# marl/l3embedding

Hardware: AMD Instinct MI355X
Metric: AVC training pairs/sec (1s audio + 224x224 frame) (higher is better)
Workload: dtype f32; 1 GPU; full cnn_L3_melspec2 AVC training step (audio+vision+fusion, fwd+bwd+Adam), batch 64 per GPU, global batch 64, fp32, inputs resident in HBM; global_batch=64, parallelism=dp1, fp32_conv=f4x4

## Files before the change

include/l3hip.h:

```cpp
#ifndef L3HIP_H
#define L3HIP_H

#include <stdint.h>

#ifdef __cplusplus
extern "C" {
#endif

#define L3_OK 0
#define L3_EINVAL (-1)
#define L3_EHIP (-2)
#define L3_ENOMEM (-3)
#define L3_ESTATE (-4)
#define L3_ECOMM (-5)

#define L3_MODEL_CNN_L3_ORIG 0
#define L3_MODEL_TINY_L3 1
#define L3_MODEL_CNN_L3_KAPREDBINPUTBN 2
#define L3_MODEL_CNN_L3_MELSPEC1 3
#define L3_MODEL_CNN_L3_MELSPEC2 4

typedef struct l3_engine l3_engine;

#define L3_DTYPE_F32 0
// ... 37 lines not shown
int l3_copy_state(l3_engine *dst, l3_engine *src);
int l3_optimizer_steps(const l3_engine *e, int64_t *adam_t, int64_t *bn_steps);

int l3_forward(l3_engine *e, const float *video, const float *audio, int training,
               float *probs, float *logits);

int l3_train_step(l3_engine *e, const float *video, const float *audio,
                  const float *labels, float lr, float *loss, float *acc);
int l3_eval_step(l3_engine *e, const float *video, const float *audio,
                 const float *labels, float *loss, float *acc);

int l3_upload_batch(l3_engine *e, const float *video, const float *audio, const float *labels);
int l3_upload_batch_raw(l3_engine *e, const uint8_t *video_u8, const int16_t *audio_i16,
                        const int32_t *labels_i32);
int l3_stage_batch_raw(l3_engine *e, const uint8_t *video_u8, const int16_t *audio_i16, const int32_t *labels_i32);
typedef struct l3_augment_params {
    int32_t start_x, start_y;
    int32_t flip;
    int32_t sat_first;
    float saturation;
    float brightness;
} l3_augment_params;
int l3_upload_batch_raw_aug(l3_engine *e, const uint8_t *video_u8, const int16_t *audio_i16, const int32_t *labels_i32,
                            const l3_augment_params *params, const double *u);
int l3_stage_batch_raw_aug(l3_engine *e, const uint8_t *video_u8, const int16_t *audio_i16, const int32_t *labels_i32,
                           const l3_augment_params *params, const double *u);
int l3_batch_gains(l3_engine *e, double *gains);
int l3_step_forward(l3_engine *e, int training);
int l3_tower_step(l3_engine *e, int tower, int backward);
int l3_step_bucket_count(const l3_engine *e);
int l3_step_backward_bucket(l3_engine *e, int bucket);
int l3_step_update(l3_engine *e, float lr, float grad_scale);
int l3_step_resident(l3_engine *e, float lr);
int l3_step_results(l3_engine *e, float *loss, float *acc, float *probs, float *logits);
int l3_step_results_enqueue(l3_engine *e, int slot, int reduce);
int l3_step_results_wait(l3_engine *e, int slot, float *loss, float *acc);

#define L3_COMM_ID_BYTES 128
int l3_comm_unique_id(void *id128);
int l3_comm_init(l3_engine *e, const void *id128, int world, int rank);
int l3_comm_destroy(l3_engine *e);
int l3_comm_info(const l3_engine *e, int *world, int *rank, char *library_path, int path_cap);
int l3_comm_version(void);
int l3_comm_allreduce_host(l3_engine *e, double *vals, int n, int op);
int l3_step_dp(l3_engine *e, float lr);
int l3_comm_timing(l3_engine *e, int on);
int l3_comm_timing_read(l3_engine *e, double *exposed_ms, double *span_ms, double *bucket_ms, int cap, int *steps);

int l3_grad_arena_dev(l3_engine *e, void **dev_ptr, int64_t *numel);
int l3_bucket_range(const l3_engine *e, int bucket, int64_t *offset, int64_t *numel);
int l3_bn_stats_pack_dev(l3_engine *e, void **send_dev, int64_t *numel);
int l3_bn_stats_replicas_dev(l3_engine *e, int world, void **gathered_dev);

int l3_embed_audio(l3_engine *e, const float *audio, int64_t n, int pool_h, int pool_w, float *out);
int l3_embed_vision(l3_engine *e, const float *video, int64_t n, int pool_h, int pool_w, float *out);
int64_t l3_embed_dim(const l3_engine *e, int vision, int pool_h, int pool_w);
int l3_embed_audio_frames(l3_engine *e, const float *samples, int64_t n_samples, const int64_t *table,
                          int64_t n_frames, int pool_h, int pool_w, float *out);
int l3_embed_audio_clips_resampled(l3_engine *e, const float *native, int64_t n_native, const int64_t *clips,
                                   int64_t n_clips, const double *half_window, int64_t n_window, int num_table,
                                   int64_t n_samples, const int64_t *table, int64_t n_frames, int pool_h, int pool_w,
                                   float *out);

int l3_get_activation(l3_engine *e, const char *name, float *dst, int64_t numel);
int l3_activation_numel(l3_engine *e, const char *name, int64_t *numel);
int l3_sync(l3_engine *e);
int l3_profile_enable(l3_engine *e, int on);
int l3_set_tower_overlap(l3_engine *e, int on);
int l3_profile_read(l3_engine *e, int family, double *ms, int64_t *launches, double *flops);
int l3_profile_read_executed(l3_engine *e, int family, double *flops);
int l3_profile_read_bytes(l3_engine *e, int family, double *bytes);

#define L3_OP_BF16_STORED 2
#define L3_OP_BF16_STORED_OUT 3
int l3_op_conv2d_fwd_dt(int device, int dtype, const float *x, const float *w, const float *b, float *y,
                        int n, int h, int wd, int cin, int cout, int kh, int kw, int same);
int l3_op_conv2d_bwd_dt(int device, int dtype, const float *x, const float *w, const float *dy, float *dx,
                        float *dw, float *db, int n, int h, int wd, int cin, int cout, int kh, int kw, int same);
int l3_op_conv2d_fwd(int device, const float *x, const float *w, const float *b, float *y,
                     int n, int h, int wd, int cin, int cout, int kh, int kw, int same);
int l3_op_conv2d_bwd(int device, const float *x, const float *w, const float *dy,
                     float *dx, float *dw, float *db,
                     int n, int h, int wd, int cin, int cout, int kh, int kw, int same);
int l3_op_bn_relu_fwd(int device, const float *x, const float *gamma, const float *beta,
                      float *y, float *mean, float *var, int64_t rows, int c, int relu, int x_bf16);
int l3_op_bn_relu_bwd(int device, const float *x, const float *y, const float *dy,
                      const float *gamma, const float *beta, const float *mean, const float *var,
                      float *dx, float *dgamma, float *dbeta, int64_t rows, int c, int relu, int x_bf16);
int l3_op_bn_relu_pool2_fwd(int device, const float *x, const float *gamma, const float *beta, float *p,
                            float *mean, float *var, int n, int h, int wd, int c, int same, int relu_mode, int x_bf16);
int l3_op_bn_relu_pool2_bwd(int device, const float *x, const float *gamma, const float *beta, const float *dp,
                            float *dx, float *dgamma, float *dbeta, float *dbias, int n, int h, int wd, int c,
                            int same, int relu_mode, int x_bf16);
int l3_op_maxpool_fwd(int device, const float *x, float *y, int n, int h, int wd, int c,
                      int ph, int pw, int sh, int sw, int same);
int l3_op_maxpool_bwd(int device, const float *x, const float *dy, float *dx, int n, int h,
                      int wd, int c, int ph, int pw, int sh, int sw, int same);
int l3_op_frontend(int device, int model_type, const float *audio, int n, int db_max_scope, float *out);
int l3_op_gather_frames(int device, const float *samples, int64_t n_samples, const int64_t *table,
                        int64_t n_frames, float *frames);
int l3_op_resample(int device, const float *x, int64_t n_in, int64_t sr_orig, int64_t sr_new, const double *half_window,
                   int64_t n_window, int num_table, int64_t t0, int64_t n_out, float *y);
int l3_op_resample_clips(int device, const float *x, int64_t n_in, const int64_t *clips, int64_t n_clips, int64_t sr_new,
                         const double *half_window, int64_t n_window, int num_table, int64_t n_samples, int copy_equal,
                         float *y);
int l3_op_bn_stats_from_partials(int device, const float *part, int nblk, int c, const float *pivot, int64_t rows,
                                 float eps, float *mean, float *var);
int l3_op_preprocess(int device, const uint8_t *video_u8, int64_t nv, float *video,
                     const int16_t *audio_i16, int64_t na, float *audio);
int l3_op_augment_video(int device, const uint8_t *u8, int n, int h, int w, const l3_augment_params *params,
                        uint8_t *out_u8, float *out_f32);
int l3_op_augment_audio(int device, const int16_t *i16, int n, int t, const double *u, int16_t *out_i16, float *out_f32,
                        double *gains);

typedef struct l3_mlp l3_mlp;
int l3_mlp_create(int device, int D, int C, int batch, float weight_decay, uint64_t seed, l3_mlp **m);
void l3_mlp_destroy(l3_mlp *m);
int64_t l3_mlp_param_count(const l3_mlp *m);
int l3_mlp_set_data(l3_mlp *m, const float *X_train, const int32_t *y_train, int64_t n_train,
                    const float *X_valid, const int32_t *y_valid, int64_t n_valid);
int l3_mlp_epoch(l3_mlp *m, const int32_t *perm, float lr, int64_t t0, double *stats_out);
int l3_mlp_predict(l3_mlp *m, const float *X, int64_t n, float *probs_out);
int l3_mlp_get_weights(l3_mlp *m, float *dst, int64_t n);
int l3_mlp_set_weights(l3_mlp *m, const float *src, int64_t n);

int l3_op_mlp_dense_fwd(int device, const float *x, int64_t n_x, const int32_t *idx, int rows, int K, int N, const float *w,
                        const float *b, int relu, float *y);
int l3_op_mlp_dense_bwd_x(int device, const float *dy, const float *w, const float *h, int rows, int K, int N, float *dx);
int l3_op_mlp_wgrad(int device, const float *x, int64_t n_x, const int32_t *idx, int rows, int K, int N, const float *dy, float *dw,
                    float *db);
int l3_op_mlp_wgrad_adam(int device, const float *x, int64_t n_x, const int32_t *idx, int rows, int K, int N, const float *dy,
                         float *w, float *b, float *mw, float *vw, float *mb, float *vb, float weight_decay, float lr_t,
                         float *w2_out);
int l3_op_mlp_softmax_ce(int device, const float *z, const int32_t *labels, int rows, int C, float gscale, float *probs, float *dz,
                         float *ce, float *correct);
int l3_op_adam(int device, float *p, const float *g, float *m, float *v, int64_t n, int64_t n_l2, float l2x2, float lr_t);
int l3_op_adam_scaled(int device, float *p, const float *g, float *m, float *v, int64_t n, int64_t n_l2, float l2x2, float lr_t,
                      float b1, float b2, float eps, float gscale);

int l3_op_head_dense_fwd(int device, const float *x, const float *w, const float *b, float *y, int B, int K, int N, int relu);
int l3_op_head_dense_bwd(int device, const float *x, const float *w, const float *dy, float *dw, float *db, float *dx, int B,
                         int K, int N);
int l3_op_softmax_ce2(int device, const float *logits, const float *labels, int B, float gscale, float *probs, float *dlogits,
                      float *stats);
int l3_op_sumsq(int device, const float *base, int64_t n_base, const int64_t *off, const int64_t *n, int count, int multi,
                float *out);
int l3_op_bn_moving_update(int device, int entries, const int32_t *c, const int64_t *slot_off, int64_t n_slots, float *moving,
                           float *biased, const float *batch, const float *gathered, int64_t n_gathered, int replicas,
                           int64_t stride, float momentum, int zero_debias, int64_t step, float *packed, int64_t n_packed);

#define L3_SVM_LINEAR 0
#define L3_SVM_POLY 1
#define L3_SVM_RBF 2
#define L3_SVM_SIGMOID 3
#define L3_SVM_DEFAULT_WS 64
#define L3_SVM_LOCAL_REL 0.1
typedef struct l3_svm_kernel {
    int32_t kind, degree;
    double gamma, coef0;
} l3_svm_kernel;
typedef struct l3_svm l3_svm;
int l3_svm_create(int device, l3_svm **m);
void l3_svm_destroy(l3_svm *m);
int l3_svm_set_data(l3_svm *m, const float *X, int64_t n, int D);
int l3_svm_fit(l3_svm *m, const l3_svm_kernel *k, double C, double tol, int64_t max_iter, int n_prob, const int64_t *prob_off,
               const int32_t *rows, const int8_t *signs, int q, double *alpha_out, double *rho_out, int64_t *updates_out,
// ... 113 lines not shown
```

l3embedding_amd/_lib.py:

```python
import ctypes as C
import os

import numpy as np

from . import _build

MODEL_IDS = {
    'cnn_L3_orig': 0,
    'tiny_L3': 1,
    'cnn_L3_kapredbinputbn': 2,
    'cnn_L3_melspec1': 3,
    'cnn_L3_melspec2': 4,
}

FAMILIES = ('conv_fwd', 'conv_dgrad', 'conv_wgrad', 'elementwise', 'frontend', 'head', 'adam')


DTYPES = {'f32': 0, 'fp32': 0, 'float32': 0, 'bf16': 1}
FP32_CONV = {'f4x4': 0, 'f2x2': 1, 'f2x2_bf16x6': 2}
DP_MOVING = {'replicas': 0, 'rank_local': 1}
OP_DTYPES = dict(DTYPES, bf16_stored=2, bf16_stored_out=3)


class L3Config(C.Structure):
# ... 10 lines not shown
        ('fp32_conv', C.c_int32),
        ('dp_moving', C.c_int32),
    ]


class L3Error(RuntimeError):
    pass


_f32p = C.POINTER(C.c_float)
_lib = None
TORCH_LOADED_FIRST = None

SIGNATURES = {
    'l3_create': (C.c_int, [C.POINTER(L3Config), C.c_uint64, C.POINTER(C.c_void_p)]),
    'l3_destroy': (None, [C.c_void_p]),
    'l3_last_error': (C.c_char_p, [C.c_void_p]),
    'l3_build_experiments': (C.c_int, []),
    'l3_comm_version': (C.c_int, []),
    'l3_bn_stats_pack_dev': (C.c_int, [C.c_void_p, C.POINTER(C.c_void_p), C.POINTER(C.c_int64)]),
    'l3_bn_stats_replicas_dev': (C.c_int, [C.c_void_p, C.c_int, C.POINTER(C.c_void_p)]),
    'l3_model_type_from_name': (C.c_int, [C.c_char_p]),
    'l3_device_count': (C.c_int, []),
    'l3_param_count': (C.c_int, [C.c_void_p]),
    'l3_param_info': (C.c_int, [C.c_void_p, C.c_int, C.c_char_p, C.c_int, C.POINTER(C.c_int32),
                                C.POINTER(C.c_int64), C.POINTER(C.c_int32), C.POINTER(C.c_int64)]),
    'l3_set_param': (C.c_int, [C.c_void_p, C.c_char_p, C.c_void_p, C.c_int64]),
    'l3_get_param': (C.c_int, [C.c_void_p, C.c_char_p, C.c_void_p, C.c_int64]),
    'l3_get_grad': (C.c_int, [C.c_void_p, C.c_char_p, C.c_void_p, C.c_int64]),
    'l3_reset_optimizer': (C.c_int, [C.c_void_p]),
    'l3_copy_state': (C.c_int, [C.c_void_p, C.c_void_p]),
    'l3_optimizer_steps': (C.c_int, [C.c_void_p, C.POINTER(C.c_int64), C.POINTER(C.c_int64)]),
    'l3_forward': (C.c_int, [C.c_void_p, C.c_void_p, C.c_void_p, C.c_int, C.c_void_p, C.c_void_p]),
    'l3_train_step': (C.c_int, [C.c_void_p, C.c_void_p, C.c_void_p, C.c_void_p, C.c_float,
                                C.POINTER(C.c_float), C.POINTER(C.c_float)]),
    'l3_eval_step': (C.c_int, [C.c_void_p, C.c_void_p, C.c_void_p, C.c_void_p,
                               C.POINTER(C.c_float), C.POINTER(C.c_float)]),
    'l3_upload_batch': (C.c_int, [C.c_void_p, C.c_void_p, C.c_void_p, C.c_void_p]),
    'l3_upload_batch_raw': (C.c_int, [C.c_void_p, C.c_void_p, C.c_void_p, C.c_void_p]),
    'l3_tower_step': (C.c_int, [C.c_void_p, C.c_int, C.c_int]),
    'l3_stage_batch_raw': (C.c_int, [C.c_void_p, C.c_void_p, C.c_void_p, C.c_void_p]),
    'l3_upload_batch_raw_aug': (C.c_int, [C.c_void_p, C.c_void_p, C.c_void_p, C.c_void_p, C.c_void_p, C.c_void_p]),
    'l3_stage_batch_raw_aug': (C.c_int, [C.c_void_p, C.c_void_p, C.c_void_p, C.c_void_p, C.c_void_p, C.c_void_p]),
    'l3_batch_gains': (C.c_int, [C.c_void_p, C.c_void_p]),
    'l3_step_forward': (C.c_int, [C.c_void_p, C.c_int]),
    'l3_step_bucket_count': (C.c_int, [C.c_void_p]),
    'l3_step_backward_bucket': (C.c_int, [C.c_void_p, C.c_int]),
    'l3_step_update': (C.c_int, [C.c_void_p, C.c_float, C.c_float]),
    'l3_step_resident': (C.c_int, [C.c_void_p, C.c_float]),
    'l3_step_results': (C.c_int, [C.c_void_p, C.POINTER(C.c_float), C.POINTER(C.c_float), C.c_void_p, C.c_void_p]),
    'l3_step_results_enqueue': (C.c_int, [C.c_void_p, C.c_int, C.c_int]),
    'l3_step_results_wait': (C.c_int, [C.c_void_p, C.c_int, C.POINTER(C.c_float), C.POINTER(C.c_float)]),
    'l3_comm_unique_id': (C.c_int, [C.c_void_p]),
    'l3_comm_init': (C.c_int, [C.c_void_p, C.c_void_p, C.c_int, C.c_int]),
    'l3_comm_destroy': (C.c_int, [C.c_void_p]),
    'l3_comm_info': (C.c_int, [C.c_void_p, C.POINTER(C.c_int), C.POINTER(C.c_int), C.c_char_p, C.c_int]),
    'l3_comm_allreduce_host': (C.c_int, [C.c_void_p, C.POINTER(C.c_double), C.c_int, C.c_int]),
    'l3_step_dp': (C.c_int, [C.c_void_p, C.c_float]),
    'l3_comm_timing': (C.c_int, [C.c_void_p, C.c_int]),
    'l3_comm_timing_read': (C.c_int, [C.c_void_p, C.POINTER(C.c_double), C.POINTER(C.c_double), C.POINTER(C.c_double), C.c_int, C.POINTER(C.c_int)]),
    'l3_grad_arena_dev': (C.c_int, [C.c_void_p, C.POINTER(C.c_void_p), C.POINTER(C.c_int64)]),
    'l3_bucket_range': (C.c_int, [C.c_void_p, C.c_int, C.POINTER(C.c_int64), C.POINTER(C.c_int64)]),
    'l3_embed_audio': (C.c_int, [C.c_void_p, C.c_void_p, C.c_int64, C.c_int, C.c_int, C.c_void_p]),
    'l3_embed_vision': (C.c_int, [C.c_void_p, C.c_void_p, C.c_int64, C.c_int, C.c_int, C.c_void_p]),
    'l3_embed_dim': (C.c_int64, [C.c_void_p, C.c_int, C.c_int, C.c_int]),
    'l3_embed_audio_frames': (C.c_int, [C.c_void_p, C.c_void_p, C.c_int64, C.c_void_p, C.c_int64, C.c_int, C.c_int,
                                        C.c_void_p]),
    'l3_embed_audio_clips_resampled': (C.c_int, [C.c_void_p, C.c_void_p, C.c_int64, C.c_void_p, C.c_int64, C.c_void_p,
                                                 C.c_int64, C.c_int, C.c_int64, C.c_void_p, C.c_int64, C.c_int, C.c_int,
                                                 C.c_void_p]),
    'l3_get_activation': (C.c_int, [C.c_void_p, C.c_char_p, C.c_void_p, C.c_int64]),
    'l3_activation_numel': (C.c_int, [C.c_void_p, C.c_char_p, C.POINTER(C.c_int64)]),
    'l3_sync': (C.c_int, [C.c_void_p]),
    'l3_profile_enable': (C.c_int, [C.c_void_p, C.c_int]),
    'l3_set_tower_overlap': (C.c_int, [C.c_void_p, C.c_int]),
    'l3_profile_read_executed': (C.c_int, [C.c_void_p, C.c_int, C.POINTER(C.c_double)]),
    'l3_profile_read_bytes': (C.c_int, [C.c_void_p, C.c_int, C.POINTER(C.c_double)]),
    'l3_profile_read': (C.c_int, [C.c_void_p, C.c_int, C.POINTER(C.c_double), C.POINTER(C.c_int64),
                                  C.POINTER(C.c_double)]),
    'l3_op_conv2d_fwd': (C.c_int, [C.c_int, C.c_void_p, C.c_void_p, C.c_void_p, C.c_void_p] + [C.c_int] * 8),
    'l3_op_conv2d_fwd_dt': (C.c_int, [C.c_int, C.c_int, C.c_void_p, C.c_void_p, C.c_void_p, C.c_void_p] + [C.c_int] * 8),
    'l3_op_conv2d_bwd_dt': (C.c_int, [C.c_int, C.c_int] + [C.c_void_p] * 6 + [C.c_int] * 8),
    'l3_op_conv2d_bwd': (C.c_int, [C.c_int] + [C.c_void_p] * 6 + [C.c_int] * 8),
    'l3_op_bn_relu_fwd': (C.c_int, [C.c_int] + [C.c_void_p] * 6 + [C.c_int64, C.c_int, C.c_int, C.c_int]),
    'l3_op_bn_relu_bwd': (C.c_int, [C.c_int] + [C.c_void_p] * 10 + [C.c_int64, C.c_int, C.c_int, C.c_int]),
    'l3_op_bn_relu_pool2_fwd': (C.c_int, [C.c_int] + [C.c_void_p] * 6 + [C.c_int] * 7),
    'l3_op_bn_relu_pool2_bwd': (C.c_int, [C.c_int] + [C.c_void_p] * 8 + [C.c_int] * 7),
    'l3_op_maxpool_fwd': (C.c_int, [C.c_int, C.c_void_p, C.c_void_p] + [C.c_int] * 9),
    'l3_op_maxpool_bwd': (C.c_int, [C.c_int, C.c_void_p, C.c_void_p, C.c_void_p] + [C.c_int] * 9),
    'l3_op_frontend': (C.c_int, [C.c_int, C.c_int, C.c_void_p, C.c_int, C.c_int, C.c_void_p]),
    'l3_op_gather_frames': (C.c_int, [C.c_int, C.c_void_p, C.c_int64, C.c_void_p, C.c_int64, C.c_void_p]),
    'l3_op_resample': (C.c_int, [C.c_int, C.c_void_p, C.c_int64, C.c_int64, C.c_int64, C.c_void_p, C.c_int64, C.c_int,
                                 C.c_int64, C.c_int64, C.c_void_p]),
    'l3_op_resample_clips': (C.c_int, [C.c_int, C.c_void_p, C.c_int64, C.c_void_p, C.c_int64, C.c_int64, C.c_void_p, C.c_int64,
                                       C.c_int, C.c_int64, C.c_int, C.c_void_p]),
    'l3_op_bn_stats_from_partials': (C.c_int, [C.c_int, C.c_void_p, C.c_int, C.c_int, C.c_void_p, C.c_int64, C.c_float,
                                               C.c_void_p, C.c_void_p]),
    'l3_op_preprocess': (C.c_int, [C.c_int, C.c_void_p, C.c_int64, C.c_void_p, C.c_void_p, C.c_int64, C.c_void_p]),
    'l3_op_augment_video': (C.c_int, [C.c_int, C.c_void_p, C.c_int, C.c_int, C.c_int, C.c_void_p, C.c_void_p, C.c_void_p]),
    'l3_op_augment_audio': (C.c_int, [C.c_int, C.c_void_p, C.c_int, C.c_int, C.c_void_p, C.c_void_p, C.c_void_p, C.c_void_p]),
    'l3_mlp_create': (C.c_int, [C.c_int, C.c_int, C.c_int, C.c_int, C.c_float, C.c_uint64, C.POINTER(C.c_void_p)]),
    'l3_mlp_destroy': (None, [C.c_void_p]),
    'l3_mlp_param_count': (C.c_int64, [C.c_void_p]),
    'l3_mlp_set_data': (C.c_int, [C.c_void_p, C.c_void_p, C.c_void_p, C.c_int64, C.c_void_p, C.c_void_p, C.c_int64]),
    'l3_mlp_epoch': (C.c_int, [C.c_void_p, C.c_void_p, C.c_float, C.c_int64, C.POINTER(C.c_double)]),
    'l3_mlp_predict': (C.c_int, [C.c_void_p, C.c_void_p, C.c_int64, C.c_void_p]),
    'l3_mlp_get_weights': (C.c_int, [C.c_void_p, C.c_void_p, C.c_int64]),
    'l3_mlp_set_weights': (C.c_int, [C.c_void_p, C.c_void_p, C.c_int64]),
    'l3_op_mlp_dense_fwd': (C.c_int, [C.c_int, C.c_void_p, C.c_int64, C.c_void_p, C.c_int, C.c_int, C.c_int, C.c_void_p,
                                      C.c_void_p, C.c_int, C.c_void_p]),
    'l3_op_mlp_dense_bwd_x': (C.c_int, [C.c_int, C.c_void_p, C.c_void_p, C.c_void_p, C.c_int, C.c_int, C.c_int, C.c_void_p]),
    'l3_op_mlp_wgrad': (C.c_int, [C.c_int, C.c_void_p, C.c_int64, C.c_void_p, C.c_int, C.c_int, C.c_int, C.c_void_p,
                                  C.c_void_p, C.c_void_p]),
    'l3_op_mlp_wgrad_adam': (C.c_int, [C.c_int, C.c_void_p, C.c_int64, C.c_void_p, C.c_int, C.c_int, C.c_int, C.c_void_p]
                             + [C.c_void_p] * 6 + [C.c_float, C.c_float, C.c_void_p]),
    'l3_op_mlp_softmax_ce': (C.c_int, [C.c_int, C.c_void_p, C.c_void_p, C.c_int, C.c_int, C.c_float] + [C.c_void_p] * 4),
    'l3_op_adam': (C.c_int, [C.c_int] + [C.c_void_p] * 4 + [C.c_int64, C.c_int64, C.c_float, C.c_float]),
    'l3_op_adam_scaled': (C.c_int, [C.c_int] + [C.c_void_p] * 4 + [C.c_int64, C.c_int64] + [C.c_float] * 6),
    'l3_op_head_dense_fwd': (C.c_int, [C.c_int] + [C.c_void_p] * 4 + [C.c_int] * 4),
    'l3_op_head_dense_bwd': (C.c_int, [C.c_int] + [C.c_void_p] * 6 + [C.c_int] * 3),
    'l3_op_softmax_ce2': (C.c_int, [C.c_int, C.c_void_p, C.c_void_p, C.c_int, C.c_float] + [C.c_void_p] * 3),
    'l3_op_sumsq': (C.c_int, [C.c_int, C.c_void_p, C.c_int64, C.c_void_p, C.c_void_p, C.c_int, C.c_int, C.c_void_p]),
    'l3_op_bn_moving_update': (C.c_int, [C.c_int, C.c_int, C.c_void_p, C.c_void_p, C.c_int64] + [C.c_void_p] * 4
                               + [C.c_int64, C.c_int, C.c_int64, C.c_float, C.c_int, C.c_int64, C.c_void_p, C.c_int64]),
    'l3_svm_create': (C.c_int, [C.c_int, C.POINTER(C.c_void_p)]),
    'l3_svm_destroy': (None, [C.c_void_p]),
    'l3_svm_set_data': (C.c_int, [C.c_void_p, C.c_void_p, C.c_int64, C.c_int]),
    'l3_svm_fit': (C.c_int, [C.c_void_p, C.c_void_p, C.c_double, C.c_double, C.c_int64, C.c_int] + [C.c_void_p] * 3
                   + [C.c_int] + [C.c_void_p] * 5),
    'l3_svm_fit_costs': (C.c_int, [C.c_void_p, C.c_void_p, C.c_void_p, C.c_double, C.c_int64, C.c_int] + [C.c_void_p] * 3
                         + [C.c_int] + [C.c_void_p] * 5),
    'l3_svm_cv_decision': (C.c_int, [C.c_void_p, C.c_void_p, C.c_int] + [C.c_void_p] * 8),
    'l3_op_svm_sigmoid_train': (C.c_int, [C.c_int, C.c_int] + [C.c_void_p] * 6),
    'l3_svm_decision': (C.c_int, [C.c_void_p, C.c_void_p, C.c_void_p, C.c_void_p, C.c_int64, C.c_int, C.c_void_p, C.c_void_p,
                                  C.c_int64, C.c_int] + [C.c_void_p] * 4),
    'l3_op_svm_kernel_rows': (C.c_int, [C.c_int, C.c_void_p, C.c_void_p, C.c_int64, C.c_int, C.c_void_p, C.c_int, C.c_void_p,
                                        C.c_int, C.c_void_p]),
    'l3_op_svm_smo': (C.c_int, [C.c_int, C.c_void_p, C.c_void_p, C.c_int, C.c_double, C.c_double, C.c_double, C.c_int64,
                                C.c_void_p, C.c_void_p, C.c_void_p]),
    'l3_svm_set_data_dev': (C.c_int, [C.c_void_p, C.c_void_p, C.c_int64, C.c_int64]),
    'l3_svm_get_rows': (C.c_int, [C.c_void_p, C.c_void_p, C.c_int64, C.c_void_p]),
    'l3_svm_set_model': (C.c_int, [C.c_void_p, C.c_void_p, C.c_void_p, C.c_void_p, C.c_int64, C.c_int, C.c_int] + [C.c_void_p] * 5),
    'l3_svm_score': (C.c_int, [C.c_void_p, C.c_void_p, C.c_void_p, C.c_void_p, C.c_int64, C.c_int64, C.c_int64, C.c_int, C.c_void_p,
                               C.c_void_p, C.c_int64] + [C.c_void_p] * 6),
    'l3_op_svm_tail': (C.c_int, [C.c_int, C.c_void_p, C.c_int64, C.c_int, C.c_void_p, C.c_void_p, C.c_void_p, C.c_void_p, C.c_int64]
                       + [C.c_void_p] * 8),
    'l3_vggish_create': (C.c_int, [C.c_int, C.c_int, C.POINTER(C.c_void_p)]),
    'l3_vggish_destroy': (None, [C.c_void_p]),
    'l3_vggish_batch': (C.c_int, [C.c_void_p]),
    'l3_vggish_set_conv': (C.c_int, [C.c_void_p, C.c_int]),
    'l3_vggish_set_weight': (C.c_int, [C.c_void_p, C.c_char_p, C.c_void_p, C.c_int64]),
    'l3_vggish_set_pca': (C.c_int, [C.c_void_p, C.c_void_p, C.c_void_p]),
    'l3_vggish_embed_clips_resampled': (C.c_int, [C.c_void_p, C.c_void_p, C.c_int64, C.c_void_p, C.c_int64, C.c_void_p, C.c_int64,
                                                  C.c_int, C.c_int64, C.c_void_p, C.c_int64, C.c_void_p, C.c_int64, C.c_int,
                                                  C.c_void_p]),
    'l3_op_vggish_logmel': (C.c_int, [C.c_int, C.c_void_p, C.c_int64, C.c_void_p, C.c_int64, C.c_void_p]),
    'l3_op_vggish_conv1': (C.c_int, [C.c_int, C.c_void_p, C.c_int64, C.c_void_p, C.c_int64, C.c_void_p, C.c_void_p, C.c_void_p]),
    'l3_op_vggish_bias_relu': (C.c_int, [C.c_int, C.c_void_p, C.c_void_p, C.c_void_p] + [C.c_int] * 5),
    'l3_op_vggish_postprocess': (C.c_int, [C.c_int, C.c_void_p, C.c_int64, C.c_void_p, C.c_void_p, C.c_int, C.c_void_p]),
    'l3_op_vggish_conv': (C.c_int, [C.c_int, C.c_int, C.c_void_p, C.c_void_p, C.c_void_p, C.c_void_p] + [C.c_int] * 6),
    'l3_feat_create': (C.c_int, [C.c_int, C.c_void_p, C.c_int64, C.c_int64, C.POINTER(C.c_void_p)]),
    'l3_feat_destroy': (None, [C.c_void_p]),
    'l3_feat_shape': (C.c_int, [C.c_void_p, C.POINTER(C.c_int64), C.POINTER(C.c_int64)]),
    'l3_feat_download': (C.c_int, [C.c_void_p, C.c_int64, C.c_int64, C.c_void_p]),
    'l3_feat_assemble': (C.c_int, [C.c_int, C.c_void_p, C.c_int64, C.POINTER(C.c_void_p)]),
    'l3_feat_gather': (C.c_int, [C.c_void_p, C.c_void_p, C.c_int64]),
# ... 352 lines not shown
        x = np.ascontiguousarray(native, dtype=np.float32).reshape(-1)
        c = np.ascontiguousarray(clips, dtype=np.int64).reshape(-1, 6)
        w = np.ascontiguousarray(half_window, dtype=np.float64).reshape(-1)
        t = np.ascontiguousarray(table, dtype=np.int64).reshape(-1, 3)
        d = self.lib.l3_embed_dim(self.h, 0, pool[0], pool[1])
        if out is None:
            out = np.empty((t.shape[0], max(d, 0)), np.float32)
        elif out.dtype != np.float32 or not out.flags['C_CONTIGUOUS'] or out.shape != (t.shape[0], d):
            raise ValueError('out must be a C-contiguous float32 array of shape %s' % ((t.shape[0], d),))
        if x.size == 0:
            x = np.zeros(1, np.float32)[:0]
        check(self.lib.l3_embed_audio_clips_resampled(self.h, _ptr(x), x.size, _ptr(c), c.shape[0], _ptr(w), w.size,
                                                      int(num_table), int(n_samples), _ptr(t), t.shape[0], pool[0], pool[1],
                                                      _ptr(out)), self.h)
        return out

    def embed_vision(self, video, pool=(7, 7)):
        v = _f32(video)
        d = self.lib.l3_embed_dim(self.h, 1, pool[0], pool[1])
        out = np.empty((v.shape[0], d), np.float32)
        check(self.lib.l3_embed_vision(self.h, _ptr(v), v.shape[0], pool[0], pool[1], _ptr(out)), self.h)
        return out

    def activation(self, name):
        n = C.c_int64()
        check(self.lib.l3_activation_numel(self.h, name.encode(), C.byref(n)), self.h)
        out = np.empty((n.value,), np.float32)
        check(self.lib.l3_get_activation(self.h, name.encode(), _ptr(out), n.value), self.h)
        return out

    def sync(self):
        check(self.lib.l3_sync(self.h), self.h)

    def set_tower_overlap(self, on=True):
        check(self.lib.l3_set_tower_overlap(self.h, int(on)), self.h)

    def profile_enable(self, on=True):
        check(self.lib.l3_profile_enable(self.h, int(on)), self.h)

    def profile_read(self):
        out = {}
        for i, fam in enumerate(FAMILIES):
            ms, n, fl = C.c_double(), C.c_int64(), C.c_double()
            check(self.lib.l3_profile_read(self.h, i, C.byref(ms), C.byref(n), C.byref(fl)), self.h)
            ex = C.c_double()
            check(self.lib.l3_profile_read_executed(self.h, i, C.byref(ex)), self.h)
            by = C.c_double()
            check(self.lib.l3_profile_read_bytes(self.h, i, C.byref(by)), self.h)
            out[fam] = dict(ms=ms.value, launches=n.value, flops=fl.value, executed_flops=ex.value, alg_bytes=by.value)
        return out


def op_conv2d_fwd(x, w, b, same, device=0, dtype='f32'):
    lib = load()
    x, w = _f32(x), _f32(w)
    b = _f32(b)
    n, h, wd, cin = x.shape
    kh, kw, _, cout = w.shape
    ho, wo = (h, wd) if same else (h - kh + 1, wd - kw + 1)
    y = np.empty((n, ho, wo, cout), np.float32)
    if OP_DTYPES[dtype]:
        check(lib.l3_op_conv2d_fwd_dt(device, OP_DTYPES[dtype], _ptr(x), _ptr(w), _ptr(b), _ptr(y), n, h, wd, cin, cout,
                                      kh, kw, int(same)))
    else:
        check(lib.l3_op_conv2d_fwd(device, _ptr(x), _ptr(w), _ptr(b), _ptr(y), n, h, wd, cin, cout, kh, kw, int(same)))
    return y


def op_conv2d_bwd(x, w, dy, same, device=0, dtype='f32'):
    lib = load()
    x, w, dy = _f32(x), _f32(w), _f32(dy)
    n, h, wd, cin = x.shape
    kh, kw, _, cout = w.shape
    dx, dw, db = np.empty_like(x), np.empty_like(w), np.empty((cout,), np.float32)
    if OP_DTYPES[dtype]:
        check(lib.l3_op_conv2d_bwd_dt(device, OP_DTYPES[dtype], _ptr(x), _ptr(w), _ptr(dy), _ptr(dx), _ptr(dw), _ptr(db),
                                      n, h, wd, cin, cout, kh, kw, int(same)))
    else:
        check(lib.l3_op_conv2d_bwd(device, _ptr(x), _ptr(w), _ptr(dy), _ptr(dx), _ptr(dw), _ptr(db),
                                   n, h, wd, cin, cout, kh, kw, int(same)))
    return dx, dw, db


def op_bn_relu_fwd(x, gamma, beta, relu, device=0, x_bf16=False):
    lib = load()
    x = _f32(x)
    c = x.shape[-1]
    rows = x.size // c
    y = np.empty_like(x)
    mean, var = np.empty((c,), np.float32), np.empty((c,), np.float32)
    check(lib.l3_op_bn_relu_fwd(device, _ptr(x), _ptr(_f32(gamma)), _ptr(_f32(beta)), _ptr(y), _ptr(mean),
                                _ptr(var), rows, c, int(relu), int(x_bf16)))
    return y, mean, var


def op_bn_relu_bwd(x, y, dy, gamma, mean, var, relu, device=0, beta=None, x_bf16=False):
    lib = load()
    x, y, dy = _f32(x), _f32(y), _f32(dy)
    c = x.shape[-1]
    rows = x.size // c
    dx = np.empty_like(x)
    dg, db = np.empty((c,), np.float32), np.empty((c,), np.float32)
    check(lib.l3_op_bn_relu_bwd(device, _ptr(x), _ptr(y), _ptr(dy), _ptr(_f32(gamma)), _ptr(_f32(beta)), _ptr(_f32(mean)),
                                _ptr(_f32(var)), _ptr(dx), _ptr(dg), _ptr(db), rows, c, int(relu), int(x_bf16)))
    return dx, dg, db


def op_bn_relu_pool2_fwd(x, gamma, beta, same, device=0, relu_mode=1, x_bf16=False):
    lib = load()
    x = _f32(x)
    n, h, wd, c = x.shape
    p = np.empty((n, _pool_out(h, 2, 2, same), _pool_out(wd, 2, 2, same), c), np.float32)
    mean, var = np.empty((c,), np.float32), np.empty((c,), np.float32)
    check(lib.l3_op_bn_relu_pool2_fwd(device, _ptr(x), _ptr(_f32(gamma)), _ptr(_f32(beta)), _ptr(p), _ptr(mean),
                                      _ptr(var), n, h, wd, c, int(same), int(relu_mode), int(x_bf16)))
    return p, mean, var


def op_bn_relu_pool2_bwd(x, gamma, beta, dp, same, device=0, relu_mode=1, x_bf16=False):
    lib = load()
    x, dp = _f32(x), _f32(dp)
    n, h, wd, c = x.shape
    dx = np.empty_like(x)
    dg, db, dbias = (np.empty((c,), np.float32) for _ in range(3))
    check(lib.l3_op_bn_relu_pool2_bwd(device, _ptr(x), _ptr(_f32(gamma)), _ptr(_f32(beta)), _ptr(dp), _ptr(dx),
                                      _ptr(dg), _ptr(db), _ptr(dbias), n, h, wd, c, int(same), int(relu_mode), int(x_bf16)))
    return dx, dg, db, dbias


def _pool_out(h, p, s, same):
    return -(-h // s) if same else (h - p) // s + 1


def op_maxpool_fwd(x, ph, pw, sh, sw, same, device=0):
    lib = load()
    x = _f32(x)
    n, h, wd, c = x.shape
    y = np.empty((n, _pool_out(h, ph, sh, same), _pool_out(wd, pw, sw, same), c), np.float32)
    check(lib.l3_op_maxpool_fwd(device, _ptr(x), _ptr(y), n, h, wd, c, ph, pw, sh, sw, int(same)))
    return y


def op_maxpool_bwd(x, dy, ph, pw, sh, sw, same, device=0):
    lib = load()
    x, dy = _f32(x), _f32(dy)
    n, h, wd, c = x.shape
    dx = np.empty_like(x)
    check(lib.l3_op_maxpool_bwd(device, _ptr(x), _ptr(dy), _ptr(dx), n, h, wd, c, ph, pw, sh, sw, int(same)))
    return dx


def op_bn_stats_from_partials(part, pivot, rows, eps=1e-3, device=0):
    lib = load()
    part, pivot = _f32(part), _f32(pivot)
    nblk, two, c = part.shape
    assert two == 2 and pivot.shape == (c,)
    mean, var = np.empty(c, np.float32), np.empty(c, np.float32)
    check(lib.l3_op_bn_stats_from_partials(device, _ptr(part), nblk, c, _ptr(pivot), int(rows), float(eps), _ptr(mean), _ptr(var)))
    return mean, var


def op_frontend(model_type, audio, db_max_scope='sample', device=0):
    lib = load()
    a = _f32(audio)
    n = a.shape[0]
    probe = {'cnn_L3_orig': (257, 197), 'tiny_L3': (257, 198), 'cnn_L3_kapredbinputbn': (257, 197),
# ... 851 lines not shown
```

l3embedding_amd/csrc/bn_fused.hip:

```cpp
#include "kernels.h"
#include "device_common.h"

namespace l3 {



__device__ __forceinline__ void store_quad(void* base, int64_t q, f32x4 v, int obf) {
    if (obf) {
        bf16x4 h;
        h[0] = (__bf16)v.x; h[1] = (__bf16)v.y; h[2] = (__bf16)v.z; h[3] = (__bf16)v.w;
        __builtin_nontemporal_store(h, reinterpret_cast<bf16x4*>(base) + q);
    } else {
        __builtin_nontemporal_store(v, reinterpret_cast<f32x4*>(base) + q);
    }
}

template <bool XBF>
__device__ __forceinline__ f32x4 load_quad(const void* base, int64_t q) {
    if constexpr (XBF) {
        const u32x2 r = __builtin_nontemporal_load(reinterpret_cast<const u32x2*>(base) + q);
        return f32x4{__uint_as_float(r.x << 16), __uint_as_float(r.x & 0xffff0000u), __uint_as_float(r.y << 16),
                     __uint_as_float(r.y & 0xffff0000u)};
    } else {
        return __builtin_nontemporal_load(reinterpret_cast<const f32x4*>(base) + q);
    }
}

static constexpr int FB = 256;
static constexpr int FAST_MAX_BLOCKS = 1024;

bool bn_fast_ok(int C) { return C >= 4 && C <= 1024 && (C & (C - 1)) == 0; }

static inline int fast_blocks(int64_t work_items) {
    int64_t b = (work_items + FB * 8 - 1) / (FB * 8);
    if (b < 1) b = 1;
    if (b > FAST_MAX_BLOCKS) b = FAST_MAX_BLOCKS;
    return (int)b;
}

size_t bn_fast_scratch_floats(int C) { return (size_t)FAST_MAX_BLOCKS * 2 * C + 8 * (size_t)C + 64; }
const float* bn_bwd_fast_coeffs(const float* scratch, int C) { return scratch + (size_t)FAST_MAX_BLOCKS * 2 * C; }

__device__ __forceinline__ void block_write_partials(f32x4 a0, f32x4 a1, float* part, int C4) {
    __shared__ f32x4 sm0[FB];
    __shared__ f32x4 sm1[FB];
    const int t = threadIdx.x;
    sm0[t] = a0;
    sm1[t] = a1;
    __syncthreads();
    if (t < C4) {
        f32x4 s0 = sm0[t], s1 = sm1[t];
        for (int k = t + C4; k < FB; k += C4) {
            s0 += sm0[k];
            s1 += sm1[k];
        }
        const int C = C4 * 4;
        *reinterpret_cast<f32x4*>(part + ((size_t)blockIdx.x * 2 + 0) * C + t * 4) = s0;
        *reinterpret_cast<f32x4*>(part + ((size_t)blockIdx.x * 2 + 1) * C + t * 4) = s1;
    }
}

__device__ __forceinline__ f32x4 bn_pre(f32x4 x, f32x4 sc, f32x4 sh) {
    return f32x4{fmaf(x.x, sc.x, sh.x), fmaf(x.y, sc.y, sh.y), fmaf(x.z, sc.z, sh.z), fmaf(x.w, sc.w, sh.w)};
}
__device__ __forceinline__ f32x4 relu4(f32x4 v) {
    return f32x4{fmaxf(v.x, 0.f), fmaxf(v.y, 0.f), fmaxf(v.z, 0.f), fmaxf(v.w, 0.f)};
}


template <bool XBF>
__global__ __launch_bounds__(FB) void bn_stats_fast_kernel(const void* x, float* part, float* pivot_out, int64_t n4, int C4,
                                                          int prerelu) {
    const int64_t q0 = (int64_t)blockIdx.x * FB + threadIdx.x;
    const int c4 = (int)(q0 % C4);
    const f32x4 row0 = load_quad<XBF>(x, c4);
    const f32x4 pivot = prerelu ? relu4(row0) : row0;
    if (pivot_out != nullptr && q0 < C4) reinterpret_cast<f32x4*>(pivot_out)[c4] = row0;
    f32x4 a0 = {0.f, 0.f, 0.f, 0.f}, a1 = {0.f, 0.f, 0.f, 0.f};
    const int64_t stride = (int64_t)gridDim.x * FB;
    for (int64_t q = q0; q < n4; q += stride) {
        const f32x4 xv = load_quad<XBF>(x, q);
        const f32x4 d = (prerelu ? relu4(xv) : xv) - pivot;
        a0 += d;
        a1 += d * d;
    }
    block_write_partials(a0, a1, part, C4);
}

template <class G, bool PRE>
__global__ __launch_bounds__(256) void fast_final_kernel(G g, const float* part, int nblk, int C, int rpb) {
    const int lane = threadIdx.x & 63, wave = threadIdx.x >> 6;
    const int c = blockIdx.x * 4 + wave;
    if (c >= C) return;
    double s0 = 0.0, s1 = 0.0;
    for (int b = lane; b < nblk; b += 64) {
        if constexpr (PRE) {
            const double* row = reinterpret_cast<const double*>(part + (size_t)b * rpb * 2 * C);
            s0 += row[c];
            s1 += row[C + c];
        } else {
            s0 += (double)part[((size_t)b * 2 + 0) * C + c];
            s1 += (double)part[((size_t)b * 2 + 1) * C + c];
        }
    }
#pragma unroll
    for (int off = 32; off > 0; off >>= 1) {
        s0 += __shfl_xor(s0, off, 64);
        s1 += __shfl_xor(s1, off, 64);
    }
    if (lane == 0) g(c, s0, s1);
}

constexpr int PRE_BLOCKS = 256;
__global__ __launch_bounds__(256) void fast_prefinal_kernel(float* part, int nblk, int C, int rpb) {
    __shared__ double sm[256][4];
    const int t = threadIdx.x;
    const int qpr = C / 2, rpi = 256 / qpr;
    const int q = t % qpr, rr = t / qpr;
    const int r0 = blockIdx.x * rpb, r1 = blockIdx.x == gridDim.x - 1 ? nblk : r0 + rpb;
    double a[4] = {0.0, 0.0, 0.0, 0.0};
    for (int r = r0 + rr; r < r1; r += rpi) {
        const f32x4 v = *reinterpret_cast<const f32x4*>(part + (size_t)r * 2 * C + q * 4);
#pragma unroll
        for (int e = 0; e < 4; ++e) a[e] += (double)v[e];
    }
#pragma unroll
    for (int e = 0; e < 4; ++e) sm[t][e] = a[e];
    __syncthreads();
    if (t < qpr && r0 < r1) {
        for (int k = 1; k < rpi; ++k)
#pragma unroll
            for (int e = 0; e < 4; ++e) a[e] += sm[k * qpr + t][e];
        double* out = reinterpret_cast<double*>(part + (size_t)r0 * 2 * C) + q * 4;
#pragma unroll
        for (int e = 0; e < 4; ++e) out[e] = a[e];
    }
}

template <class G>
static void launch_fast_final(G g, const float* part, int nblk, int C, hipStream_t s) {
    if (nblk > 2048 && C >= 8 && C <= 512 && 256 % (C / 2) == 0 && C % 2 == 0) {
        const int rpb = (nblk + PRE_BLOCKS - 1) / PRE_BLOCKS;
        const int chunks = nblk % rpb == 1 ? nblk / rpb : (nblk + rpb - 1) / rpb;
        hipLaunchKernelGGL(fast_prefinal_kernel, dim3(chunks), dim3(256), 0, s, const_cast<float*>(part), nblk, C, rpb);
        hipLaunchKernelGGL((fast_final_kernel<G, true>), dim3((C + 3) / 4), dim3(256), 0, s, g, part, chunks, C, rpb);
        return;
    }
    hipLaunchKernelGGL((fast_final_kernel<G, false>), dim3((C + 3) / 4), dim3(256), 0, s, g, part, nblk, C, 1);
}

struct StatFinal {
    const float* x;
    const float* gamma;
    const float* beta;
    float *mean, *var, *scale, *shift;
    double inv_n;
    float eps;
    int prerelu;
    __device__ void operator()(int c, double s0, double s1) const {
        const double dm = s0 * inv_n;
        double v = s1 * inv_n - dm * dm;
        if (v < 0.0) v = 0.0;
        const double m = (double)(prerelu ? fmaxf(x[c], 0.f) : x[c]) + dm;
        mean[c] = (float)m;
        var[c] = (float)v;
        const double sc = (double)gamma[c] / sqrt(v + (double)eps);
        scale[c] = (float)sc;
        shift[c] = (float)((double)beta[c] - m * sc);
    }
};

void bn_stats_from_partials(const float* part, int nblk, const float* pivot, const float* gamma, const float* beta,
                            float* mean, float* var, float* scale, float* shift, int64_t rows, int C, float eps,
                            int prerelu, hipStream_t s) {
    launch_fast_final(StatFinal{pivot, gamma, beta, mean, var, scale, shift, 1.0 / (double)rows, eps, prerelu}, part, nblk,
                      C, s);
}

void bn_stats_fast(const float* x, const float* gamma, const float* beta, float* mean, float* var, float* scale,
                   float* shift, float* scratch, int64_t rows, int C, float eps, int prerelu, hipStream_t s, int x_bf16) {
    const int64_t n4 = rows * (C / 4);
    const int nb = fast_blocks(n4);
    if (x_bf16) {
        float* pivot = scratch + (size_t)FAST_MAX_BLOCKS * 2 * C;
        hipLaunchKernelGGL(bn_stats_fast_kernel<true>, dim3(nb), dim3(FB), 0, s, (const void*)x, scratch, pivot, n4, C / 4, prerelu);
        launch_fast_final(StatFinal{pivot, gamma, beta, mean, var, scale, shift, 1.0 / (double)rows, eps, prerelu}, scratch, nb, C, s);
        return;
    }
    hipLaunchKernelGGL(bn_stats_fast_kernel<false>, dim3(nb), dim3(FB), 0, s, (const void*)x, scratch, (float*)nullptr, n4,
                       C / 4, prerelu);
    launch_fast_final(StatFinal{x, gamma, beta, mean, var, scale, shift, 1.0 / (double)rows, eps, prerelu}, scratch, nb, C, s);
}

// ... 269 lines not shown
        constexpr int U = XBF ? 2 : 1;
        const int64_t total = (int64_t)g.N * g.Hc * g.Wc * g.C4;
        for (int64_t q = (int64_t)blockIdx.x * (FB * U) + threadIdx.x; q < total; q += stride * U) {
            f32x4 rs[U][4], dps[U];
            int64_t bases[U];
            bool w1[U], h1[U], lives[U], on[U];
#pragma unroll
            for (int u = 0; u < U; ++u) {
                on[u] = q + u * FB < total;
                int n, hc, wc;
                pool_index(g, on[u] ? q + u * FB : q, g.Hc, g.Wc, n, hc, wc);
                const int h0 = 2 * hc, w0 = 2 * wc;
                h1[u] = h0 + 1 < g.H; w1[u] = w0 + 1 < g.W;
                lives[u] = hc < g.Ho && wc < g.Wo;
                const int64_t base = ((int64_t)(n * g.H + h0) * g.W + w0) * g.C4 + c4;
                const int64_t dw = w1[u] ? g.C4 : 0, dh = h1[u] ? (int64_t)g.W * g.C4 : 0;
                bases[u] = base;
                rs[u][0] = load_quad<XBF>(x, base); rs[u][1] = load_quad<XBF>(x, base + dw);
                rs[u][2] = load_quad<XBF>(x, base + dh); rs[u][3] = load_quad<XBF>(x, base + dh + dw);
                dps[u] = f32x4{0.f, 0.f, 0.f, 0.f};
                if (lives[u]) dps[u] = load_quad<DYBF>(dy, (int64_t)n * g.out_bs4 + ((int64_t)hc * g.Wo + wc) * g.C4 + c4);
            }
#pragma unroll
            for (int u = 0; u < U; ++u) {
                if (!on[u]) continue;
                const bool h1ok = h1[u], w1ok = w1[u], live = lives[u];
                const int64_t base = bases[u];
                const int64_t dw = w1ok ? g.C4 : 0, dh = h1ok ? (int64_t)g.W * g.C4 : 0;
                const f32x4 r00 = rs[u][0], r01 = rs[u][1], r10 = rs[u][2], r11 = rs[u][3];
                f32x4 x00 = r00, x01 = r01, x10 = r10, x11 = r11;
                if (relu == 2) { x00 = relu4(x00); x01 = relu4(x01); x10 = relu4(x10); x11 = relu4(x11); }
                f32x4 d00 = {0.f, 0.f, 0.f, 0.f}, d01 = d00, d10 = d00, d11 = d00;
                if (live) {
                    f32x4 p00 = bn_pre(x00, sc, sh), p01 = bn_pre(x01, sc, sh), p10 = bn_pre(x10, sc, sh),
                          p11 = bn_pre(x11, sc, sh);
                    const float gate = relu == 2 ? -INFINITY : 0.f;
                    if (relu != 2) { p00 = relu4(p00); p01 = relu4(p01); p10 = relu4(p10); p11 = relu4(p11); }
                    const f32x4 dp = dps[u];
                    const bool ok11 = h1ok && w1ok;
#define L3_APP(comp)                                                                                      \
    {                                                                                                     \
        const int k = argmax4(p00.comp, p01.comp, p10.comp, p11.comp, w1ok, h1ok, ok11);                  \
        const float pk = k == 0 ? p00.comp : k == 1 ? p01.comp : k == 2 ? p10.comp : p11.comp;            \
        const float d = pk > gate ? dp.comp : 0.f;                                                        \
        d00.comp = k == 0 ? d : 0.f;                                                                      \
        d01.comp = k == 1 ? d : 0.f;                                                                      \
        d10.comp = k == 2 ? d : 0.f;                                                                      \
        d11.comp = k == 3 ? d : 0.f;                                                                      \
    }
                    L3_APP(x) L3_APP(y) L3_APP(z) L3_APP(w)
#undef L3_APP
                }
                auto gate2 = [&](f32x4 o, f32x4 r) {
                    if (relu == 2) {
                        o.x = r.x > 0.f ? o.x : 0.f; o.y = r.y > 0.f ? o.y : 0.f;
                        o.z = r.z > 0.f ? o.z : 0.f; o.w = r.w > 0.f ? o.w : 0.f;
                    }
                    return o;
                };
                const f32x4 o00 = gate2(A * d00 + (B * x00 + Cc), r00);
                store_quad(dx, base, o00, obf);
                a0 += o00;
                if (w1ok) {
                    const f32x4 o = gate2(A * d01 + (B * x01 + Cc), r01);
                    store_quad(dx, base + dw, o, obf);
                    a0 += o;
                }
                if (h1ok) {
                    const f32x4 o = gate2(A * d10 + (B * x10 + Cc), r10);
                    store_quad(dx, base + dh, o, obf);
                    a0 += o;
                }
                if (h1ok && w1ok) {
                    const f32x4 o = gate2(A * d11 + (B * x11 + Cc), r11);
                    store_quad(dx, base + dh + dw, o, obf);
                    a0 += o;
                }
            }
        }
    }
    if (part != nullptr) block_write_partials(a0, a0, part, g.C4);
}

struct SumFinal {
    float* out;
    __device__ void operator()(int c, double s0, double) const { out[c] = (float)s0; }
};

void bn_bwd_fast(const float* x, const float* scale, const float* shift, const float* mean, const float* var,
                 const float* gamma, const float* dy, int pooled, int N, int H, int W, int C, int Ho, int Wo,
                 int64_t dy_batch_stride, float* dx, float* dgamma, float* dbeta, float* dbias, float* scratch,
                 float eps, int relu, int training, hipStream_t s, int dx_bf16, int x_bf16, int dy_bf16,
                 const float* ready_part, int ready_blocks) {
    const int64_t rows = (int64_t)N * H * W;
    const int64_t n4 = rows * (C / 4);
    Pool2Geom g = make_pool2(N, H, W, C, pooled ? Ho : H, pooled ? Wo : W, pooled ? dy_batch_stride : (int64_t)H * W * C);
    float* part = scratch;
    float* cA = scratch + (size_t)FAST_MAX_BLOCKS * 2 * C;
    float* cB = cA + C;
    float* cC = cB + C;
    const void* xv = (const void*)x;
    const void* dyv = (const void*)dy;
    const f32x4* sc4 = reinterpret_cast<const f32x4*>(scale);
    const f32x4* sh4 = reinterpret_cast<const f32x4*>(shift);
    const int64_t work_r = pooled ? (int64_t)N * Ho * Wo * (C / 4) : n4;
    const int nb_r = fast_blocks(work_r);
    const int variant = (pooled ? 4 : 0) | (x_bf16 ? 2 : 0) | (dy_bf16 ? 1 : 0);
    using ReduceFn = void (*)(const void*, const void*, const f32x4*, const f32x4*, const f32x4*, const f32x4*, float*, int64_t,
                              Pool2Geom, float, int);
    static const ReduceFn reduce_fns[8] = {
        bn_bwd_reduce_fast_kernel<false, false, false>, bn_bwd_reduce_fast_kernel<false, false, true>,
        bn_bwd_reduce_fast_kernel<false, true, false>,  bn_bwd_reduce_fast_kernel<false, true, true>,
        bn_bwd_reduce_fast_kernel<true, false, false>,  bn_bwd_reduce_fast_kernel<true, false, true>,
        bn_bwd_reduce_fast_kernel<true, true, false>,   bn_bwd_reduce_fast_kernel<true, true, true>};
    if (ready_part != nullptr) {
        launch_fast_final(BwdFinal{gamma, mean, var, dgamma, dbeta, cA, cB, cC, 1.0 / (double)rows, eps, training}, ready_part,
                          ready_blocks, C, s);
    } else {
        hipLaunchKernelGGL(reduce_fns[variant], dim3(nb_r), dim3(FB), 0, s, xv, dyv, sc4, sh4, reinterpret_cast<const f32x4*>(mean),
                           reinterpret_cast<const f32x4*>(var), part, n4, g, eps, relu);
        launch_fast_final(BwdFinal{gamma, mean, var, dgamma, dbeta, cA, cB, cC, 1.0 / (double)rows, eps, training}, part,
                          nb_r, C, s);
    }
    if (dx == nullptr) return;
    const int64_t work_a = pooled ? (int64_t)N * g.Hc * g.Wc * (C / 4) : n4;
    const int nb_a = fast_blocks(work_a);
    float* part2 = dbias ? part : nullptr;
    using ApplyFn = void (*)(const void*, const void*, const f32x4*, const f32x4*, const f32x4*, const f32x4*, const f32x4*, void*,
                             float*, int64_t, Pool2Geom, int, int);
    static const ApplyFn apply_fns[8] = {
        bn_bwd_apply_fast_kernel<false, false, false>, bn_bwd_apply_fast_kernel<false, false, true>,
        bn_bwd_apply_fast_kernel<false, true, false>,  bn_bwd_apply_fast_kernel<false, true, true>,
        bn_bwd_apply_fast_kernel<true, false, false>,  bn_bwd_apply_fast_kernel<true, false, true>,
        bn_bwd_apply_fast_kernel<true, true, false>,   bn_bwd_apply_fast_kernel<true, true, true>};
    hipLaunchKernelGGL(apply_fns[variant], dim3(nb_a), dim3(FB), 0, s, xv, dyv, sc4, sh4, reinterpret_cast<const f32x4*>(cA),
                       reinterpret_cast<const f32x4*>(cB), reinterpret_cast<const f32x4*>(cC), (void*)dx, part2, n4, g, relu,
                       dx_bf16);
    if (dbias) launch_fast_final(SumFinal{dbias}, part, nb_a, C, s);
}

}
```

l3embedding_amd/csrc/conv.hip:

```cpp
#include "kernels.h"
#include "device_common.h"
#include <cstdlib>
#include <mutex>

namespace l3 {



struct ConvArgs {
    const float* x;
    const float* w;
    const float* bias;
    float* y;
    int N, H, W, Cin, Ho, Wo, Cout, KH, KW, padT, padL;
    int M, K, nkt, cpt;
    int mtiles, ntiles;
    int nvec;
};


__device__ __attribute__((aligned(16))) float g_zero_page[16];

template <int WAVES_M, int WAVES_N, int WT_M, int WT_N, int BKT, bool SMALLC, bool NVEC>
__global__ __launch_bounds__(256) void conv_igemm_kernel(ConvArgs a) {
// ... 660 lines not shown
    const int wave = t >> 6, lane = t & 63;
    const int wk = wave >> 1, wn = wave & 1;
    const int l31 = lane & 31, hi32 = lane >> 5;

    f32x16 acc[TKm][TNn];
#pragma unroll
    for (int i = 0; i < TKm; ++i)
#pragma unroll
        for (int j = 0; j < TNn; ++j)
#pragma unroll
            for (int r = 0; r < 16; ++r) acc[i][j][r] = 0.f;

    const int nchunks = (m_end - m_begin + WG_MC - 1) / WG_MC;
    if (nchunks > 0) {
        load_chunk(m_begin);
        store_chunk(0);
    }
    __syncthreads();
    for (int ch = 0; ch < nchunks; ++ch) {
        const int buf = ch & 1;
        const bool more = ch + 1 < nchunks;
        if (more) load_chunk(m_begin + (ch + 1) * WG_MC);
        const float* Ab = As + buf * A_TILE + hi32 * TK + wk * WK + l31;
        const float* Db = Ds + buf * D_TILE + hi32 * TN + wn * WN + l31;
#pragma unroll
        for (int s2 = 0; s2 < WG_MC / 2; ++s2) {
            float av[TKm], bv[TNn];
#pragma unroll
            for (int i = 0; i < TKm; ++i) av[i] = Ab[s2 * 2 * TK + i * 32];
#pragma unroll
            for (int j = 0; j < TNn; ++j) bv[j] = Db[s2 * 2 * TN + j * 32];
#pragma unroll
            for (int i = 0; i < TKm; ++i)
#pragma unroll
                for (int j = 0; j < TNn; ++j)
                    acc[i][j] = __builtin_amdgcn_mfma_f32_32x32x2f32(av[i], bv[j], acc[i][j], 0, 0, 0);
        }
        if (more) store_chunk(buf ^ 1);
        __syncthreads();
    }

    float* out = a.part + (size_t)sp * a.K * a.Cout;
#pragma unroll
    for (int j = 0; j < TNn; ++j) {
        const int n = n0 + wn * WN + j * 32 + l31;
#pragma unroll
        for (int i = 0; i < TKm; ++i)
#pragma unroll
            for (int r = 0; r < 16; ++r) {
                const int k = k0 + wk * WK + i * 32 + (r & 3) + 8 * (r >> 2) + 4 * hi32;
                if (n < a.Cout && k < a.K) out[(size_t)k * a.Cout + n] = acc[i][j][r];
            }
    }
}

__global__ void wgrad_reduce_kernel(const float* part, float* dw, int64_t n, int splits) {
    for (int64_t i = (int64_t)blockIdx.x * blockDim.x + threadIdx.x; i < n;
         i += (int64_t)gridDim.x * blockDim.x) {
        float s = 0.f;
        for (int sp = 0; sp < splits; ++sp) s += part[(int64_t)sp * n + i];
        dw[i] = s;
    }
}

template <int SG>
__global__ __launch_bounds__(256) void wgrad_reduce4_kernel(const f32x4* __restrict__ part, f32x4* __restrict__ dw,
                                                            int64_t n4, int splits) {
    constexpr int QPB = 256 / SG;
    __shared__ f32x4 red[256];
    const int q = threadIdx.x % QPB, g = threadIdx.x / QPB;
    const int64_t i = (int64_t)blockIdx.x * QPB + q;
    f32x4 s = {0.f, 0.f, 0.f, 0.f};
    if (i < n4)
        for (int sp = g; sp < splits; sp += SG) s += __builtin_nontemporal_load(part + (int64_t)sp * n4 + i);
    red[threadIdx.x] = s;
    __syncthreads();
    if (g == 0 && i < n4) {
#pragma unroll
        for (int k = 1; k < SG; ++k) s += red[k * QPB + q];
        dw[i] = s;
    }
}

static void wgrad_reduce(const float* part, float* dw, int64_t n, int splits, hipStream_t s) {
    if (n % 4 == 0 && splits > 1) {
        const int64_t n4 = n / 4;
        if (n4 < 1024 && splits >= 256)
            hipLaunchKernelGGL(wgrad_reduce4_kernel<64>, dim3((unsigned)((n4 + 3) / 4)), dim3(256), 0, s,
                               reinterpret_cast<const f32x4*>(part), reinterpret_cast<f32x4*>(dw), n4, splits);
        else if (n4 / 64 >= 1024 || splits < 16)
            hipLaunchKernelGGL(wgrad_reduce4_kernel<4>, dim3((unsigned)((n4 + 63) / 64)), dim3(256), 0, s,
                               reinterpret_cast<const f32x4*>(part), reinterpret_cast<f32x4*>(dw), n4, splits);
        else
            hipLaunchKernelGGL(wgrad_reduce4_kernel<16>, dim3((unsigned)((n4 + 15) / 16)), dim3(256), 0, s,
                               reinterpret_cast<const f32x4*>(part), reinterpret_cast<f32x4*>(dw), n4, splits);
        return;
    }
    const int blocks = (int)((n + 255) / 256 < 4096 ? (n + 255) / 256 : 4096);
    hipLaunchKernelGGL(wgrad_reduce_kernel, dim3(blocks), dim3(256), 0, s, part, dw, n, splits);
}

struct Wgrad9Args {
    const float* x;
    const float* dy;
    float* part;
    int N, H, W, Cin, Cout;
    int co_tiles, tiles, ph, pw;
    int npatch, per_split, splits;
};

__global__ __launch_bounds__(256) void conv_wgrad9_kernel(Wgrad9Args a) {
    constexpr int A_TILE = 36 * 64, D_TILE = 16 * 64;
    __shared__ __attribute__((aligned(16))) float smem[2 * (A_TILE + D_TILE)];
    float* As = smem;
    float* Ds = smem + 2 * A_TILE;
    const int t = threadIdx.x;
    const int logical = xcd_remap(blockIdx.x, a.tiles * a.splits);
    const int sp = logical / a.tiles, tile = logical - sp * a.tiles;
    const int cit = tile / a.co_tiles, cot = tile - cit * a.co_tiles;
    const int ci0 = cit * 64, co0 = cot * 64;
    const int p_begin = sp * a.per_split;
    const int p_end = min(a.npatch, p_begin + a.per_split);

    int hpix[3], hc4[3];
#pragma unroll
    for (int i = 0; i < 3; ++i) {
        const int f = t + 256 * i;
        hpix[i] = f >> 4;
        hc4[i] = f & 15;
    }
    const int dpix = t >> 4, dc4 = t & 15;
    const int dpy = dpix >> 2, dpx = dpix & 3;

    f32x4 areg[3], dreg;
    auto load_patch = [&](int pidx) {
        const int per_img = a.ph * a.pw;
        const int n = pidx / per_img, rem = pidx - n * per_img;
        const int py = rem / a.pw, px = rem - py * a.pw;
        const int h0 = py * 4, w0 = px * 4;
#pragma unroll
        for (int i = 0; i < 3; ++i) {
            const int hy = hpix[i] / 6, hx = hpix[i] - hy * 6;
            const int hi = h0 + hy - 1, wi = w0 + hx - 1;
            const bool ok = (i < 2 || t + 512 < 576) && (unsigned)hi < (unsigned)a.H && (unsigned)wi < (unsigned)a.W;
            const float* p = ok ? a.x + ((size_t)((n * a.H + hi) * a.W + wi) * a.Cin + ci0 + hc4[i] * 4) : g_zero_page;
            areg[i] = *reinterpret_cast<const f32x4*>(p);
        }
        {
            const int ho = h0 + dpy, wo = w0 + dpx;
            const bool ok = ho < a.H && wo < a.W;
            const float* p = ok ? a.dy + ((size_t)((n * a.H + ho) * a.W + wo) * a.Cout + co0 + dc4 * 4) : g_zero_page;
            dreg = *reinterpret_cast<const f32x4*>(p);
        }
    };
    auto store_patch = [&](int buf) {
        *reinterpret_cast<f32x4*>(&As[buf * A_TILE + t * 4]) = areg[0];
        *reinterpret_cast<f32x4*>(&As[buf * A_TILE + (t + 256) * 4]) = areg[1];
        if (t + 512 < 576) *reinterpret_cast<f32x4*>(&As[buf * A_TILE + (t + 512) * 4]) = areg[2];
        *reinterpret_cast<f32x4*>(&Ds[buf * D_TILE + t * 4]) = dreg;
    };

    const int wave = t >> 6, lane = t & 63;
    const int wk = wave >> 1, wn = wave & 1;
    const int l31 = lane & 31, hi32 = lane >> 5;

    f32x16 acc[9];
#pragma unroll
    for (int i = 0; i < 9; ++i)
#pragma unroll
        for (int r = 0; r < 16; ++r) acc[i][r] = 0.f;

    if (p_begin < p_end) {
        load_patch(p_begin);
// ... 229 lines not shown
#pragma unroll
    for (int tap = 0; tap < 9; ++tap)
#pragma unroll
        for (int r = 0; r < 16; ++r) {
            const int k = tap * a.Cin + ci0 + wk * 32 + (r & 3) + 8 * (r >> 2) + 4 * hi32;
            out[(size_t)k * a.Cout + n] = acc[tap][r];
        }
}

static bool wgrad9_ok(const ConvGeom& g) {
    return g.KH == 3 && g.KW == 3 && g.padT == 1 && g.padL == 1 && g.Ho == g.H && g.Wo == g.W && g.Cin % 64 == 0 &&
           g.Cout % 64 == 0;
}

struct Wgrad9Plan {
    int tiles, co_tiles, ph, pw, npatch, per_split, splits;
};
static Wgrad9Plan wgrad9_plan(const ConvGeom& g) {
    Wgrad9Plan p;
    p.co_tiles = g.Cout / 64;
    p.tiles = (g.Cin / 64) * p.co_tiles;
    p.ph = (g.H + 3) / 4;
    p.pw = (g.W + 3) / 4;
    p.npatch = g.N * p.ph * p.pw;
    static int target = l3_knob("L3_WG9_BLOCKS") ? atoi(l3_knob("L3_WG9_BLOCKS")) : 512;
    int splits = (target + p.tiles - 1) / p.tiles;
    const int max_splits = (p.npatch + 15) / 16;
    if (splits > max_splits) splits = max_splits;
    if (splits < 1) splits = 1;
    p.per_split = (p.npatch + splits - 1) / splits;
    p.splits = (p.npatch + p.per_split - 1) / p.per_split;
    return p;
}

struct WgradPlan {
    int TK, TN, ktiles, ntiles, splits, m_per_split;
    bool smallc;
};

static WgradPlan wgrad_plan(const ConvGeom& g) {
    WgradPlan p;
    const int K = g.KH * g.KW * g.Cin, M = g.N * g.Ho * g.Wo;
    p.smallc = (g.Cin % 64) != 0;
    p.TK = (!p.smallc && g.Cin % 128 == 0) ? 128 : 64;
    p.TN = g.Cout > 64 ? 128 : 64;
    p.ktiles = (K + p.TK - 1) / p.TK;
    p.ntiles = (g.Cout + p.TN - 1) / p.TN;
    const int tiles = p.ktiles * p.ntiles;
    int splits = (1024 + tiles - 1) / tiles;
    const int max_splits = (M + 255) / 256 > 0 ? (M + 255) / 256 : 1;
    if (splits > max_splits) splits = max_splits;
    if (splits < 1) splits = 1;
    int mps = (M + splits - 1) / splits;
    mps = (mps + WG_MC - 1) / WG_MC * WG_MC;
    p.m_per_split = mps;
    p.splits = (M + mps - 1) / mps;
    return p;
}

static int wgrad9_chunk_samples(const ConvGeom& g) {
    const size_t per_sample = (size_t)g.H * g.W * (g.Cin > g.Cout ? g.Cin : g.Cout) * 4;
    size_t nc = ((1ull << 31) - 1 - (size_t)(g.W + 1) * g.Cin * 4) / per_sample;
    if (nc > (size_t)g.N) nc = (size_t)g.N;
    return nc < 1 ? 1 : (int)nc;
}
static int wgrad9_total_splits(const ConvGeom& g) {
    const int nc = wgrad9_chunk_samples(g);
    int total = 0;
    for (int n0 = 0; n0 < g.N; n0 += nc) {
        ConvGeom gc = g;
        gc.N = g.N - n0 < nc ? g.N - n0 : nc;
        total += wgrad9_plan(gc).splits;
    }
    return total;
}

static int wgw_total_splits(const ConvGeom& g) {
    const int nc = wgrad9_chunk_samples(g);
    int total = 0;
    for (int n0 = 0; n0 < g.N; n0 += nc) total += conv_wgrad_wino_max_splits(g, g.N - n0 < nc ? g.N - n0 : nc);
    return total;
}

size_t conv_wgrad_scratch_floats(const ConvGeom& g) {
    if (wgrad9_ok(g)) {
        const size_t direct = (size_t)wgrad9_total_splits(g) * 9 * g.Cin * g.Cout;
        const size_t wino = ((size_t)wgw_total_splits(g) + 1) * 16 * g.Cin * g.Cout;
        return direct > wino ? direct : wino;
    }
    const WgradPlan p = wgrad_plan(g);
    const size_t generic = (size_t)p.splits * g.KH * g.KW * g.Cin * g.Cout, first = conv_first_wgrad_scratch_floats(g);
    return generic > first ? generic : first;
}

bool conv_wgrad_bf16_ok(const ConvGeom& g) {
    return wgrad9_ok(g) && (size_t)g.H * g.W * (g.Cin > g.Cout ? g.Cin : g.Cout) * 4 + (size_t)(g.W + 1) * g.Cin * 4 < (1ull << 31);
}

double conv_wgrad_executed_flops(const ConvGeom& g, bool bf16) {
    if (!bf16 && wgrad9_ok(g) && conv_wgrad_bf16_ok(g) && conv_wgrad_wino_ok(g)) return conv_wgrad_wino_executed_flops(g);
    return -1.0;
}

void conv_wgrad(const float* x, const float* dy, float* dw, float* part, const ConvGeom& g,
                hipStream_t s, bool bf16, bool in_bf16, const FirstWgFuse* first_fuse) {
    if (wgrad9_ok(g)) {
        static const int use_t = l3_knob("L3_WG9T") ? atoi(l3_knob("L3_WG9T")) : 1;
        const bool fits = conv_wgrad_bf16_ok(g);
        if (!bf16 && fits && conv_wgrad_wino_ok(g)) {
            const int nc = wgrad9_chunk_samples(g);
            const size_t slice = (size_t)16 * g.Cin * g.Cout;
            int total = 0;
            for (int n0 = 0; n0 < g.N; n0 += nc) {
                const int n = g.N - n0 < nc ? g.N - n0 : nc;
                conv_wgrad_wino_launch(x + (size_t)n0 * g.H * g.W * g.Cin, dy + (size_t)n0 * g.H * g.W * g.Cout,
                                       part + (size_t)total * slice, g, n, s);
                total += conv_wgrad_wino_splits(g, n);
            }
            float* sum = part + (size_t)total * slice;
            if (total > 1) wgrad_reduce(part, sum, (int64_t)slice, total, s);
            conv_wgrad_wino_finish(total > 1 ? sum : part, dw, g, 1, s);
            return;
        }
        const int nc = fits ? wgrad9_chunk_samples(g) : g.N;
        const size_t slice = (size_t)9 * g.Cin * g.Cout;
        int total_splits = 0;
        for (int n0 = 0; n0 < g.N; n0 += nc) {
            ConvGeom gc = g;
            gc.N = g.N - n0 < nc ? g.N - n0 : nc;
            const Wgrad9Plan p = wgrad9_plan(gc);
            Wgrad9Args a;
            const size_t es = in_bf16 ? 2 : 4;
            a.x = reinterpret_cast<const float*>(reinterpret_cast<const char*>(x) + (size_t)n0 * g.H * g.W * g.Cin * es);
            a.dy = reinterpret_cast<const float*>(reinterpret_cast<const char*>(dy) + (size_t)n0 * g.H * g.W * g.Cout * es);
            a.part = part + (size_t)total_splits * slice;
            a.N = gc.N; a.H = g.H; a.W = g.W; a.Cin = g.Cin; a.Cout = g.Cout;
            a.co_tiles = p.co_tiles; a.tiles = p.tiles; a.ph = p.ph; a.pw = p.pw;
            a.npatch = p.npatch; a.per_split = p.per_split; a.splits = p.splits;
            constexpr size_t WG9T_LDS = 2 * (64 * 50 + 64 * 18) * sizeof(float);
            if (bf16 && fits && in_bf16 && conv_wgrad_bf16_tr_enabled()) {
                conv_wgrad_bf16_tr_launch(a.x, a.dy, a.part, g, gc.N, p.splits, s);
            } else if (bf16 && fits && in_bf16) {
                static std::once_flag once[L3_MAX_DEVICES];
                int dev = 0;
                (void)hipGetDevice(&dev);
                std::call_once(once[dev & (L3_MAX_DEVICES - 1)], [] {
                    (void)hipFuncSetAttribute((const void*)conv_wgrad9t_kernel<true, true>,
                                              hipFuncAttributeMaxDynamicSharedMemorySize, (int)(2 * WG9T_LDS));
                });
                hipLaunchKernelGGL((conv_wgrad9t_kernel<true, true>), dim3(p.tiles * p.splits), dim3(256), 2 * WG9T_LDS, s, a);
            } else if (bf16 && fits) {
                hipLaunchKernelGGL(conv_wgrad9t_kernel<true>, dim3(p.tiles * p.splits), dim3(256), WG9T_LDS, s, a);
            } else if (use_t && fits) {
                hipLaunchKernelGGL(conv_wgrad9t_kernel<false>, dim3(p.tiles * p.splits), dim3(256), WG9T_LDS, s, a);
            } else {
                hipLaunchKernelGGL(conv_wgrad9_kernel, dim3(p.tiles * p.splits), dim3(256), 0, s, a);
            }
            total_splits += p.splits;
        }
        wgrad_reduce(part, dw, (int64_t)slice, total_splits, s);
        return;
    }
    if (!bf16 && conv_first_wgrad_ok(g)) {
        const int parts = conv_first_wgrad(x, dy, part, g, s, first_fuse);
        wgrad_reduce(part, dw, (int64_t)g.KH * g.KW * g.Cin * g.Cout, parts, s);
        return;
    }
    const WgradPlan p = wgrad_plan(g);
    WgradArgs a;
    a.x = x; a.dy = dy; a.part = part;
    a.N = g.N; a.H = g.H; a.W = g.W; a.Cin = g.Cin; a.Ho = g.Ho; a.Wo = g.Wo; a.Cout = g.Cout;
    a.KH = g.KH; a.KW = g.KW; a.padT = g.padT; a.padL = g.padL;
    a.M = g.N * g.Ho * g.Wo;
    a.K = g.KH * g.KW * g.Cin;
    a.ktiles = p.ktiles; a.ntiles = p.ntiles; a.splits = p.splits; a.m_per_split = p.m_per_split;
    a.nvec = (g.Cout % 4) == 0;
    dim3 grid(p.ktiles * p.ntiles, p.splits), block(256);
#define L3_WG(TK_, TN_, SC_)                                                                              \
    do {                                                                                                  \
        if (a.nvec)                                                                                       \
            hipLaunchKernelGGL((conv_wgrad_kernel<TK_, TN_, SC_, true>), grid, block, 0, s, a);           \
        else                                                                                              \
            hipLaunchKernelGGL((conv_wgrad_kernel<TK_, TN_, SC_, false>), grid, block, 0, s, a);          \
    } while (0)
    if (p.smallc) {
        if (p.TN == 128) L3_WG(64, 128, true); else L3_WG(64, 64, true);
    } else if (p.TK == 128) {
        if (p.TN == 128) L3_WG(128, 128, false); else L3_WG(128, 64, false);
    } else {
        if (p.TN == 128) L3_WG(64, 128, false); else L3_WG(64, 64, false);
    }
#undef L3_WG
    wgrad_reduce(part, dw, (int64_t)a.K * a.Cout, p.splits, s);
}

}
```

l3embedding_amd/csrc/conv_path.h:

```cpp
#pragma once
#include "kernels.h"

namespace l3 {

ConvGeom conv_geom(int n, int h, int w, int cin, int cout, int kh, int kw, bool same, int f2x2);
ConvGeom conv_dgrad_geom(const ConvGeom& g);

struct ConvStorage {
    bool mixed = false;
    bool x_bf16 = false, y_bf16 = false, dy_bf16 = false, dx_bf16 = false;
};

enum ConvFwd { CF_BF16_STORED, CF_BF16_CAST, CF_FIRST, CF_FP32 };
enum ConvWgrad { WG_BF16_STORED, WG_BF16_CAST, WG_FP32 };
enum ConvDgrad { DG_NONE, DG_SMALL, DG_BF16_STORED, DG_BF16_CAST, DG_WINO, DG_FLIPPED };
struct ConvFwdPath {
    ConvFwd path = CF_FP32;
    bool wino_filter = false;
    double executed = -1.0;
};
struct ConvWgradPath {
    ConvWgrad path = WG_FP32;
    double executed = -1.0;
};
struct ConvDgradPath {
    ConvDgrad path = DG_NONE;
    double executed = -1.0;
};
ConvFwdPath conv_resolve_fwd(const ConvGeom& g, const ConvStorage& st, bool have_u);
ConvWgradPath conv_resolve_wgrad(const ConvGeom& g, const ConvStorage& st);
ConvDgradPath conv_resolve_dgrad(const ConvGeom& g, const ConvGeom& dg, const ConvStorage& st, bool have_u);

struct ConvBufs {
    const float* x = nullptr;
    const float* w = nullptr;
    const float* bias = nullptr;
    float* y = nullptr;
    float* dx = nullptr;
    float* dw = nullptr;
    float* wprep = nullptr;
    float* wino_u = nullptr;
    bool u_ready = false;
    float* wg_part = nullptr;
    float* stat_part = nullptr;
    int stat_mode = 0;
    const BnBwdFuse* bn_bwd = nullptr;
};
void conv_run_fwd(const ConvFwdPath& p, const ConvGeom& g, const ConvStorage& st, const ConvBufs& b, hipStream_t s);
void conv_run_wgrad(const ConvWgradPath& p, const ConvGeom& g, const ConvBufs& b, hipStream_t s);
void conv_run_dgrad(const ConvDgradPath& p, const ConvGeom& g, const ConvGeom& dg, const ConvStorage& st, const ConvBufs& b, hipStream_t s);

}
```

l3embedding_amd/csrc/conv_path.hip:

```cpp
#include "conv_path.h"

namespace l3 {

ConvGeom conv_geom(int n, int h, int w, int cin, int cout, int kh, int kw, bool same, int f2x2) {
    ConvGeom g{n, h, w, cin, 0, 0, cout, kh, kw, 0, 0};
    if (same) {
        tf_same(h, kh, 1, &g.Ho, &g.padT);
        tf_same(w, kw, 1, &g.Wo, &g.padL);
    } else {
        g.Ho = h - kh + 1;
        g.Wo = w - kw + 1;
    }
    g.f2x2 = f2x2;
    return g;
}

ConvGeom conv_dgrad_geom(const ConvGeom& g) {
    ConvGeom dg{g.N, g.Ho, g.Wo, g.Cout, g.H, g.W, g.Cin, g.KH, g.KW, g.KH - 1 - g.padT, g.KW - 1 - g.padL};
    dg.f2x2 = g.f2x2;
    dg.solo = g.solo;
    return dg;
}

ConvFwdPath conv_resolve_fwd(const ConvGeom& g, const ConvStorage& st, bool have_u) {
    ConvFwdPath p;
    const bool mp = st.mixed && conv_bf16_ok(g);
    p.path = mp ? (st.x_bf16 ? CF_BF16_STORED : CF_BF16_CAST) : conv_first_ok(g) ? CF_FIRST : CF_FP32;
    p.wino_filter = have_u && !mp && conv_wino_ok(g);
    p.executed = p.wino_filter ? conv_wino_executed_flops(g) : -1.0;
    return p;
}

ConvWgradPath conv_resolve_wgrad(const ConvGeom& g, const ConvStorage& st) {
    ConvWgradPath p;
    const bool wbf = st.mixed && conv_wgrad_bf16_ok(g);
    p.path = !wbf ? WG_FP32 : st.x_bf16 && st.dy_bf16 ? WG_BF16_STORED : WG_BF16_CAST;
    p.executed = conv_wgrad_executed_flops(g, wbf);
    return p;
}

ConvDgradPath conv_resolve_dgrad(const ConvGeom& g, const ConvGeom& dg, const ConvStorage& st, bool have_u) {
    ConvDgradPath p;
    const bool dbf = st.mixed && conv_bf16_ok(dg), wino = have_u && conv_wino_ok(dg);
    p.path = conv_dgrad_small_ok(g) ? DG_SMALL : dbf ? (st.dy_bf16 ? DG_BF16_STORED : DG_BF16_CAST) : wino ? DG_WINO : DG_FLIPPED;
    p.executed = wino && !dbf ? conv_wino_executed_flops(dg) : -1.0;
    return p;
}

void conv_run_fwd(const ConvFwdPath& p, const ConvGeom& g, const ConvStorage& st, const ConvBufs& b, hipStream_t s) {
    if (p.wino_filter && !b.u_ready) conv_wino_transform_weights(b.w, b.wino_u, g, false, s);
    switch (p.path) {
        case CF_BF16_STORED:
            conv_weights_bf16(b.w, b.wprep, g.KH, g.KW, g.Cin, g.Cout, true, s);
            conv_bf16_fwd(b.x, b.wprep, b.bias, b.y, g, s, true, b.stat_part, b.stat_mode, st.y_bf16);
            break;
        case CF_BF16_CAST:
            conv_flip_weights(b.w, b.wprep, g.KH, g.KW, g.Cin, g.Cout, s);
            conv_bf16_fwd(b.x, b.wprep, b.bias, b.y, g, s);
            break;
        case CF_FIRST:
            conv_first_fwd(b.x, b.w, b.bias, b.y, g, s, b.stat_part, b.stat_mode, st.y_bf16);
            break;
        case CF_FP32:
            conv_fwd(b.x, b.w, b.bias, b.y, g, s, p.wino_filter ? b.wino_u : nullptr, b.stat_part, b.stat_mode);
            break;
    }
}

void conv_run_wgrad(const ConvWgradPath& p, const ConvGeom& g, const ConvBufs& b, hipStream_t s) {
    conv_wgrad(b.x, b.y, b.dw, b.wg_part, g, s, p.path != WG_FP32, p.path == WG_BF16_STORED);
}

void conv_run_dgrad(const ConvDgradPath& p, const ConvGeom& g, const ConvGeom& dg, const ConvStorage& st, const ConvBufs& b, hipStream_t s) {
    switch (p.path) {
        case DG_SMALL:
            (void)conv_dgrad_small(b.y, b.w, b.dx, g, s);
            break;
        case DG_BF16_STORED:
            conv_weights_bf16(b.w, b.wprep, g.KH, g.KW, g.Cin, g.Cout, false, s);
            conv_bf16_fwd(b.y, b.wprep, nullptr, b.dx, dg, s, true, b.stat_part, 0, st.dx_bf16, b.bn_bwd);
            break;
        case DG_BF16_CAST:
            conv_bf16_fwd(b.y, b.w, nullptr, b.dx, dg, s);
            break;
        case DG_WINO:
            conv_wino_transform_weights(b.w, b.wino_u, dg, true, s);
            conv_fwd(b.y, nullptr, nullptr, b.dx, dg, s, b.wino_u, b.stat_part, 0, b.bn_bwd);
            break;
        case DG_FLIPPED:
            conv_flip_weights(b.w, b.wprep, g.KH, g.KW, g.Cin, g.Cout, s);
            conv_fwd(b.y, b.wprep, nullptr, b.dx, dg, s);
            break;
        case DG_NONE: break;
    }
}

}
```

l3embedding_amd/csrc/conv_wgrad_wino.hip:

```cpp
#include "kernels.h"
#include "device_common.h"
#include "wgw_common.h"

#include <stdlib.h>

#include <mutex>

namespace l3 {

namespace {

__device__ __forceinline__ f32x2 lds_f32x2(unsigned lds_offset) {
    const f32x2 v = *reinterpret_cast<const __attribute__((address_space(3))) f32x2*>((uintptr_t)lds_offset);
    asm volatile("");
    return v;
}

__device__ __forceinline__ f32x2 pk_fma(f32x2 c, f32x2 x, f32x2 y) {
    asm("v_pk_fma_f32 %0, %1, %2, %0" : "+v"(y) : "s"(c), "v"(x));
    return y;
}
__device__ __forceinline__ f32x2 pk_fma_w(f32x2 c, f32x2 x, f32x2 y) {
    asm("v_pk_fma_f32 %0, %1, %2, %0\n\ts_nop 3" : "+v"(y) : "s"(c), "v"(x));
    return y;
}
template <int UC>
__global__ __launch_bounds__(1024) void conv_wgrad_wino_kernel(WgwArgs a) {
    using G = WgwGeom<UC>;
    constexpr int UR = G::UR, XPITCH = G::XPITCH, YPITCH = G::YPITCH;
    extern __shared__ __attribute__((aligned(16))) char smem[];

    const int t = threadIdx.x;
    const int wave = __builtin_amdgcn_readfirstlane(t >> 6), lane = t & 63;
    const int tiles = a.ctiles * a.ktiles;
    const int logical = xcd_remap(blockIdx.x, tiles * a.splits);
    const int sp = logical / tiles, tile = logical - sp * tiles;
    const int ct = tile / a.ktiles, kt = tile - ct * a.ktiles;
    const int c0 = ct * 64, k0 = kt * 64;
    const int u_begin = sp * a.per_split, u_end = min(a.units, u_begin + a.per_split);

    unsigned pc_voff[2], pc_out[2];
    bool pc_isx[2];
    const int y_last = 2 * UR * (a.uy - 1), x_last = 2 * UC * (a.ux - 1);
#pragma unroll
    for (int q = 0; q < 2; ++q) {
        const int piece = wave + 16 * q;
        const bool isx = piece < G::XPIECES;
        const int pix = (isx ? piece : piece - G::XPIECES) * 4 + (lane >> 4);
        const int pitch = isx ? XPITCH : YPITCH;
        const int py = pix / pitch, px = pix - py * pitch;
        const int C = isx ? a.Cin : a.Cout;
        const int ry = py - (isx ? 1 : 0), rx = px - (isx ? 1 : 0);
        pc_isx[q] = isx;
        pc_voff[q] = (unsigned)((py * a.W + px) * C * 4 + (isx ? c0 : k0) * 4 + (lane & 15) * 16);
        unsigned out = 0;
#pragma unroll
        for (int cls = 0; cls < 16; ++cls) {
            const int rc = cls >> 2, cc = cls & 3;
            const bool bad = ((rc & 1) && ry < 0) || ((rc & 2) && y_last + ry >= a.H) || ((cc & 1) && rx < 0) ||
                             ((cc & 2) && x_last + rx >= a.W) || (isx && pix >= G::XPIX);
            out |= bad ? 1u << cls : 0u;
        }
        pc_out[q] = out;
    }
    const bool second = wave + 16 < G::PIECES;
    const size_t xshift = (size_t)(a.W + 1) * a.Cin * 4;
    const __amdgpu_buffer_rsrc_t xsrd = __builtin_amdgcn_make_buffer_rsrc(
        (void*)(reinterpret_cast<const char*>(a.x) - xshift), 0, (int)((size_t)a.N * a.H * a.W * a.Cin * 4 + xshift), 0x00020000);
    const __amdgpu_buffer_rsrc_t ysrd =
        __builtin_amdgcn_make_buffer_rsrc((void*)a.dy, 0, (int)((size_t)a.N * a.H * a.W * a.Cout * 4), 0x00020000);

    const int per_img = a.uy * a.ux;
    int un = u_begin / per_img;
    int uyi = (u_begin - un * per_img) / a.ux;
    int uxi = u_begin - un * per_img - uyi * a.ux;

    auto issue = [&](int buf) {
        const int Y0 = 2 * UR * uyi, X0 = 2 * UC * uxi;
        const int xbase = ((un * a.H + Y0) * a.W + X0) * a.Cin * 4;
        const int ybase = ((un * a.H + Y0) * a.W + X0) * a.Cout * 4;
        const int rcls = (1 - min(uyi, 1)) + 2 * (1 - min(a.uy - 1 - uyi, 1)), ccls = (1 - min(uxi, 1)) + 2 * (1 - min(a.ux - 1 - uxi, 1));
        const int cls = rcls * 4 + ccls;
        char* S = smem + buf * G::STAGE;
#pragma unroll
        for (int q = 0; q < 2; ++q) {
// ... 68 lines not shown
        }
        const f32x2 xc = lds_f32x2(p_ab + sb + ix), xd = lds_f32x2(p_bb + sb + ix);
        f32x2 ya = lds_f32x2(q_00 + sb + iy), yb = ya, yc = ya, yd = ya;
        if (NC == 2) yb = lds_f32x2(q_01 + sb + iy);
        if (NR == 2) yc = lds_f32x2(q_10 + sb + iy);
        if (NR == 2 && NC == 2) yd = lds_f32x2(q_11 + sb + iy);
        r.x[0] = xa; r.x[1] = xb; r.x[2] = xc; r.x[3] = xd;
        r.y[0] = ya; r.y[1] = yb; r.y[2] = yc; r.y[3] = yd;
    };
    auto mfma_step = [&](const Raw& r) {
        const f32x2 v = pk_fma_w(sb2, pk_fma(sa2, r.x[3], r.x[2]), pk_fma(sa2, r.x[1], r.x[0]));
        f32x2 z;
        if constexpr (NR == 1 && NC == 1) {
            z = r.y[0];
        } else if constexpr (NR == 1) {
            z = pk_fma_w(w01_2, r.y[1], r.y[0]);
        } else if constexpr (NC == 1) {
            z = pk_fma_w(w10_2, r.y[2], r.y[0]);
        } else {
            z = pk_fma_w(w11_2, r.y[3], pk_fma(w10_2, r.y[2], pk_fma(w01_2, r.y[1], r.y[0])));
        }
#pragma unroll
        for (int i = 0; i < 2; ++i)
#pragma unroll
            for (int jn = 0; jn < 2; ++jn) acc[i][jn] = __builtin_amdgcn_mfma_f32_32x32x2f32(v[i], z[jn], acc[i][jn], 0, 0, 0);
    };
    auto compute = [&](auto BUF) {
        constexpr int S = decltype(BUF)::value * G::STAGE;
        Raw r0, r1;
        load_raw(S, std::integral_constant<int, 0>{}, r0, r0);
        __builtin_amdgcn_sched_barrier(0);
        load_raw(S, std::integral_constant<int, 1>{}, r1, r0);
        mfma_step(r0);
        __builtin_amdgcn_sched_barrier(0);
        load_raw(S, std::integral_constant<int, 2>{}, r0, r1);
        mfma_step(r1);
        __builtin_amdgcn_sched_barrier(0);
        load_raw(S, std::integral_constant<int, 3>{}, r1, r0);
        mfma_step(r0);
        __builtin_amdgcn_sched_barrier(0);
        mfma_step(r1);
    };
    auto stage_barrier = [&]() {
        __builtin_amdgcn_sched_barrier(0);
        __syncthreads();
        __builtin_amdgcn_sched_barrier(0);
    };

    const int nunits = u_end - u_begin;
    if (nunits > 0) {
        issue(0);
        __syncthreads();
        for (int u = 0; u < nunits; u += 2) {
            if (u + 1 < nunits) issue(1);
            compute(std::integral_constant<int, 0>{});
            stage_barrier();
            if (u + 1 < nunits) {
                if (u + 2 < nunits) issue(0);
                compute(std::integral_constant<int, 1>{});
                stage_barrier();
            }
        }
    }
    };
    if (nr == 1 && nc == 1)
        run(std::integral_constant<int, 1>{}, std::integral_constant<int, 1>{});
    else if (nr == 1)
        run(std::integral_constant<int, 1>{}, std::integral_constant<int, 2>{});
    else if (nc == 1)
        run(std::integral_constant<int, 2>{}, std::integral_constant<int, 1>{});
    else
        run(std::integral_constant<int, 2>{}, std::integral_constant<int, 2>{});

    float* out = a.part + ((size_t)(sp * 16 + xi * 4 + nu) * a.Cin + c0) * a.Cout + k0;
#pragma unroll
    for (int i = 0; i < 2; ++i)
#pragma unroll
        for (int r = 0; r < 16; ++r) {
            const int c = 2 * ((r & 3) + 8 * (r >> 2) + 4 * half) + i;
            __builtin_nontemporal_store(f32x2{w00 * acc[i][0][r], w00 * acc[i][1][r]}, reinterpret_cast<f32x2*>(out + (size_t)c * a.Cout + 2 * l31));
        }
}

__global__ __launch_bounds__(256) void wgw_finish_kernel(const float* __restrict__ part, float* __restrict__ dw, int cc,
                                                         int splits) {
    const int idx = blockIdx.x * 256 + threadIdx.x;
    if (idx >= cc) return;
    float u[16];
#pragma unroll
    for (int p = 0; p < 16; ++p) u[p] = 0.f;
    for (int s = 0; s < splits; ++s)
#pragma unroll
        for (int p = 0; p < 16; ++p) u[p] += __builtin_nontemporal_load(part + ((size_t)s * 16 + p) * cc + idx);
    float rrow[3][4];
#pragma unroll
    for (int nu = 0; nu < 4; ++nu) {
        const float h1 = 0.5f * u[4 + nu], h2 = 0.5f * u[8 + nu];
        rrow[0][nu] = u[nu] + (h1 + h2);
        rrow[1][nu] = h1 - h2;
        rrow[2][nu] = (h1 + h2) + u[12 + nu];
    }
#pragma unroll
    for (int kh = 0; kh < 3; ++kh) {
        const float h1 = 0.5f * rrow[kh][1], h2 = 0.5f * rrow[kh][2];
        dw[(size_t)(kh * 3 + 0) * cc + idx] = rrow[kh][0] + (h1 + h2);
        dw[(size_t)(kh * 3 + 1) * cc + idx] = h1 - h2;
        dw[(size_t)(kh * 3 + 2) * cc + idx] = (h1 + h2) + rrow[kh][3];
    }
}

struct WgwPlan {
    int uc, uy, ux, units, per_split, splits;
};

WgwPlan wgw_plan(const ConvGeom& g, int n, int force_uc = 0) {
    const int TY = (g.H + 1) / 2, TX = (g.W + 1) / 2;
    WgwPlan p;
    size_t best = ~(size_t)0;
    p.uc = 8;
    for (int uc : {8, 4, 2}) {
        const int ur = 8 / uc;
        const size_t padded = (size_t)((TY + ur - 1) / ur * ur) * ((TX + uc - 1) / uc * uc);
        if (padded < best) {
            best = padded;
            p.uc = uc;
        }
    }
    const char* fenv = l3_knob("L3_WGW_UC");
    const int force = force_uc ? force_uc : fenv ? atoi(fenv) : 0;
    if (force == 8 || force == 4 || force == 2) p.uc = force;
    const int ur = 8 / p.uc;
    p.uy = (TY + ur - 1) / ur;
    p.ux = (TX + p.uc - 1) / p.uc;
    p.units = n * p.uy * p.ux;
    const int tiles = (g.Cin / 64) * (g.Cout / 64);
    static const int target = l3_knob("L3_WGW_BLOCKS") ? atoi(l3_knob("L3_WGW_BLOCKS")) : 256;
    int splits = (target + tiles - 1) / tiles;
    const int max_splits = (p.units + 31) / 32;
    if (splits > max_splits) splits = max_splits;
    if (splits < 1) splits = 1;
    p.per_split = (p.units + splits - 1) / splits;
    p.splits = (p.units + p.per_split - 1) / p.per_split;
    return p;
}

template <int UC>
void launch_wgw(const WgwArgs& a, hipStream_t s) {
    using G = WgwGeom<UC>;
    static std::once_flag once[L3_MAX_DEVICES];
    int dev = 0;
    (void)hipGetDevice(&dev);
    std::call_once(once[dev & (L3_MAX_DEVICES - 1)], [] {
        (void)hipFuncSetAttribute((const void*)conv_wgrad_wino_kernel<UC>, hipFuncAttributeMaxDynamicSharedMemorySize,
                                  (int)G::LDS_BYTES);
    });
    hipLaunchKernelGGL((conv_wgrad_wino_kernel<UC>), dim3(a.ctiles * a.ktiles * a.splits), dim3(1024), G::LDS_BYTES, s, a);
}

}

bool conv_wgrad_wino_ok(const ConvGeom& g) {
    const char* env = l3_knob("L3_WG_WINO");
    return (env ? atoi(env) : 1) && g.KH == 3 && g.KW == 3 && g.padT == 1 && g.padL == 1 && g.Ho == g.H && g.Wo == g.W &&
           g.Cin % 64 == 0 && g.Cout % 64 == 0;
}

int conv_wgrad_wino_splits(const ConvGeom& g, int n) { return wgw_plan(g, n).splits; }

int conv_wgrad_wino_max_splits(const ConvGeom& g, int n) {
    int m = wgw_plan(g, n).splits;
    for (int uc : {8, 4, 2}) {
        const int sp = wgw_plan(g, n, uc).splits;
        if (sp > m) m = sp;
    }
    return m;
}

double conv_wgrad_wino_executed_flops(const ConvGeom& g) {
    const WgwPlan p = wgw_plan(g, g.N);
    return 2.0 * 16.0 * (double)p.units * 8.0 * (double)g.Cin * (double)g.Cout;
}

void conv_wgrad_wino_launch(const float* x, const float* dy, float* part, const ConvGeom& g, int n, hipStream_t s) {
    const WgwPlan p = wgw_plan(g, n);
    WgwArgs a;
    a.x = x; a.dy = dy; a.part = part;
    a.N = n; a.H = g.H; a.W = g.W; a.Cin = g.Cin; a.Cout = g.Cout;
    a.uy = p.uy; a.ux = p.ux; a.units = p.units; a.per_split = p.per_split; a.splits = p.splits;
    a.ctiles = g.Cin / 64; a.ktiles = g.Cout / 64;
#ifdef L3_EXPERIMENTS
    const char* bx = l3_knob("L3_WG_BX6");
    if (bx != nullptr && atoi(bx) == 1) return conv_wgrad_bx6_launch(a, p.uc, s);
#endif
    if (p.uc == 8)
        launch_wgw<8>(a, s);
    else if (p.uc == 4)
        launch_wgw<4>(a, s);
    else
        launch_wgw<2>(a, s);
}

void conv_wgrad_wino_finish(const float* part, float* dw, const ConvGeom& g, int splits, hipStream_t s) {
    const int cc = g.Cin * g.Cout;
    hipLaunchKernelGGL(wgw_finish_kernel, dim3((cc + 255) / 256), dim3(256), 0, s, part, dw, cc, splits);
}

}
```

l3embedding_amd/csrc/engine.hip:

```cpp
#include <hip/hip_runtime.h>
#include "knobs.h"

#include <cmath>
#include <cstdio>
#include <cstdlib>
#include <cstring>
#include <map>
#include <string>
#include <vector>

#include "../../include/l3hip.h"
#include "comm.h"
#include "conv_path.h"
#include "kernels.h"

namespace {

using namespace l3;

static thread_local std::string g_create_error;

constexpr float BN_EPS = 1e-3f;
constexpr float BN_MOMENTUM = 0.99f;
constexpr float L2_WEIGHT = 1e-5f;
constexpr float ADAM_B1 = 0.9f, ADAM_B2 = 0.999f, ADAM_EPS = 1e-8f;
constexpr int AUDIO_T = 48000;

enum ParamKind { PK_KERNEL, PK_BIAS, PK_GAMMA, PK_BETA, PK_MMEAN, PK_MVAR, PK_CONST };
enum OpKind { OP_CONV, OP_BN, OP_RELU, OP_POOL, OP_FLATTEN };
enum Family { F_CONV_FWD, F_CONV_DGRAD, F_CONV_WGRAD, F_ELEMWISE, F_FRONTEND, F_HEAD, F_ADAM, F_COUNT };

struct Tensor {
    float* d = nullptr;
    float* g = nullptr;
    int N = 0, H = 0, W = 0, C = 0;
    int64_t batch_stride = 0;
    bool alias = false;
    bool d_bf16 = false, g_bf16 = false;
    int64_t numel() const { return (int64_t)N * H * W * C; }
    int64_t rows() const { return (int64_t)N * H * W; }
};

struct Param {
    std::string name;
    int ndim = 0;
    int64_t shape[4] = {1, 1, 1, 1};
    bool trainable = false;
    int kind = 0;
    int64_t numel = 0;
    int bucket = 0;
    float* d = nullptr;
    float* g = nullptr;
};

enum FirstWgrad { FW_NONE, FW_AUG, FW_AUG_DEFERRED };
struct ConvPlan {
    ConvStorage st;
    ConvFwdPath fwd;
    int stat_mode = 0;
    FirstWgrad aug = FW_NONE;
    ConvWgradPath wgrad;
    bool colsum = false;
    ConvDgradPath dgrad;
    int bwd_bn = -1;
    double fwd_bytes = 0.0, wg_bytes = 0.0, dg_bytes = 0.0;
};
enum BnStats { BS_PARTIALS, BS_FAST, BS_PLAIN, BS_MOVING };
enum BnBwd { BB_BY_FIRST_CONV, BB_FAST_POOLED, BB_FAST, BB_FAST_DEFERRED, BB_PLAIN };
struct BnPlan {
    BnStats stats = BS_MOVING;
    int stat_blocks = 0;
    BnBwd bwd = BB_PLAIN;
    int bwd_blocks = 0;
    double fwd_bytes = 0.0, bwd_bytes = 0.0;
};

struct Op {
    OpKind kind;
    std::string name;
    int in = 0, out = 0;
    int block = 0, bucket = 0;
    int kh = 0, kw = 0, cout = 0;
    bool same = false;
    ConvGeom geom{};
    ConvGeom dgeom{};
    int p_kernel = -1, p_bias = -1;
    float* wflip = nullptr;
    float *wino_uf = nullptr, *wino_ud = nullptr;
    int in_bn = -1;
    bool fused_first = false;
    bool defer_apply = false;
    int bn_defer = -1;
    float *xaug = nullptr, *gaug = nullptr;
    ConvGeom ageom{};
    int bn_follow = -1;
    bool need_dx = true;
    int dy_to_bn = -1;
    float* xwin = nullptr;
    int p_gamma = -1, p_beta = -1, p_mmean = -1, p_mvar = -1;
    bool fused_relu = false;
    bool prerelu = false;
    int fuse_pool = -1;
    int bias_param = -1;
    bool fused_into_bn = false;
    bool bias_by_bn = false;
    float *mean = nullptr, *var = nullptr, *scale = nullptr, *shift = nullptr;
    float *biased_mean = nullptr, *biased_var = nullptr;
    PoolGeom pg{};
    ConvPlan cp{};
    BnPlan bp{};
};

struct Tower {
    std::string prefix;
    std::vector<Tensor> t;
    std::vector<Op> ops;
    int nblocks = 0;
    int emb_conv_op = -1;
    bool training = false;
};

struct FrontendDef {
    int n_dft, n_hop, same, n_mels, sqrt_out, db, loglambda;
    const char* layer_name;
};

struct ProfRec {
    int family;
    hipEvent_t a, b;
    double flops;
    double executed;
    double bytes;
    const char* tag;
};

}

struct l3_engine {
    l3_config cfg{};
    int B = 0;
    hipStream_t stream = nullptr;
    bool own_stream = false;
    hipStream_t side = nullptr;
    hipEvent_t ev_fork = nullptr, ev_join = nullptr;
    float *red_scratch2 = nullptr, *wg_scratch2 = nullptr;
    float *stat_scratch = nullptr, *stat_scratch2 = nullptr;
    size_t stat_max = 0;
    float* w4_tail = nullptr;
    bool overlap = true;
    BnMovingEntry* bn_table = nullptr;
    int bn_table_n = 0, bn_table_max_c = 0;
    std::string err;
    l3::DeviceBufs bufs;

    std::vector<Param> params;
    std::map<std::string, int> pindex;
    float *arena_p = nullptr, *arena_g = nullptr, *arena_m = nullptr, *arena_v = nullptr;
    int64_t n_train = 0;
    struct Segment { int64_t off, n; bool l2; };
    std::vector<Segment> segments;
    struct Bucket { int64_t off, n; };
    std::vector<Bucket> buckets;
    int64_t adam_t = 0;
    int64_t bn_step = 0;

    Tower vis, aud;
    FrontendDef fe{};
    FrontendCfg fcfg{};
    int p_real = -1, p_imag = -1, p_mel = -1;
    bool consts_dirty = true;
    float *wdft = nullptr, *melw = nullptr, *frames = nullptr, *spec = nullptr, *smax = nullptr;
    bool dft_consts_done = false;
    float *dft_win = nullptr, *dft_b1 = nullptr, *dft_b2 = nullptr, *dft_tw = nullptr, *dft_y = nullptr, *dft_a2 = nullptr, *dft_nyq = nullptr;
    int *mel_start = nullptr, *mel_len = nullptr, *mel_off = nullptr;
    int64_t melw_cap = 0;

    float *video = nullptr, *audio = nullptr, *labels = nullptr;
    uint8_t* raw_video = nullptr;
    int16_t* raw_audio = nullptr;
    int32_t* raw_labels = nullptr;
    uint8_t* nxt_video = nullptr;
    int16_t* nxt_audio = nullptr;
    int32_t* nxt_labels = nullptr;
    hipStream_t copy_stream = nullptr;
    hipEvent_t ev_staged = nullptr, ev_adopted = nullptr;
    float* res_host = nullptr;
    float* res_sum = nullptr;
    bool res_reduced[2] = {false, false};
    bool res_pending[2] = {false, false};
    hipEvent_t ev_res[2] = {nullptr, nullptr};
// ... 937 lines not shown
        if (f.db) db_normalize(e->aud.t[0].d, e->smax, B, e->aud.t[0].batch_stride, e->cfg.db_max_scope, e->stream);
    }
    return L3_OK;
}

static inline double act_bytes(const Tensor& t) { return (double)t.numel() * (t.d_bf16 ? 2.0 : 4.0); }
static inline double grad_bytes(const Tensor& t) { return (double)t.numel() * (t.g_bf16 ? 2.0 : 4.0); }

int plan_tower(l3_engine* e, Tower& tw, bool training, int solo) {
    static const int epi_stats = knob_int("L3_EPILOGUE_STATS", 1);
    const bool bf16 = e->cfg.dtype == L3_DTYPE_BF16;
    tw.training = training;
    auto fits = [&](const Op& cv, int blocks, int C) {
        if ((size_t)blocks * 2 * C <= e->stat_max) return true;
        e->err = cv.name + ": " + std::to_string(blocks) + " partial blocks of " + std::to_string(C) + " channels exceed the statistics scratch (" +
                 std::to_string(e->stat_max) + " floats)";
        return false;
    };
    auto defers = [&](const Op& bn) {
        return training && bn.defer_apply && bn.fuse_pool < 0 && bn_fast_ok(tw.t[bn.in].C) && tw.t[bn.in].d_bf16 == tw.t[bn.out].g_bf16;
    };
    for (auto& op : tw.ops) op.bp = BnPlan{};
    for (auto& op : tw.ops) {
        if (op.kind != OP_CONV) continue;
        op.geom.solo = op.dgeom.solo = solo;
        op.geom.dynamic = op.dgeom.dynamic = e->comm != nullptr ? 1 : 0;
        float* ts = solo ? e->w4_tail : nullptr;
        op.geom.tail_scratch = op.dgeom.tail_scratch = ts;
        op.geom.tail_scratch_bytes = op.dgeom.tail_scratch_bytes = ts ? conv_wino4_tail_scratch_bytes() : 0;

        const Tensor &x = tw.t[op.in], &y = tw.t[op.out];
        const double wbytes = (double)e->params[op.p_kernel].numel * 4.0;
        ConvPlan& p = op.cp = ConvPlan{};
        p.st = ConvStorage{bf16, x.d_bf16, y.d_bf16, y.g_bf16, x.g_bf16};
        p.fwd = conv_resolve_fwd(op.geom, p.st, op.wino_uf != nullptr);
        p.fwd_bytes = act_bytes(x) + act_bytes(y) + wbytes;
        const int nblk = p.fwd.path == CF_BF16_STORED ? conv_bf16_stat_blocks(op.geom)
                         : p.fwd.path == CF_FIRST     ? conv_first_stat_blocks(op.geom)
                         : p.fwd.path == CF_FP32 && p.fwd.wino_filter ? conv_wino_stat_blocks(op.geom) : 0;
        if (epi_stats && training && op.bn_follow >= 0 && e->stat_max > 0 && nblk > 0) {
            if (!fits(op, nblk, op.geom.Cout)) return L3_ESTATE;
            p.stat_mode = tw.ops[op.bn_follow].prerelu ? 2 : 1;
            tw.ops[op.bn_follow].bp.stat_blocks = nblk;
        }
        if (training && op.in_bn >= 0) {
            const Op* fb = op.bn_defer >= 0 && defers(tw.ops[op.bn_defer]) ? &tw.ops[op.bn_defer] : nullptr;
            p.aug = fb ? FW_AUG_DEFERRED : FW_AUG;
            p.wg_bytes = (double)x.rows() * op.ageom.Cin * 4.0 + (fb ? act_bytes(tw.t[fb->in]) + grad_bytes(tw.t[fb->out]) : grad_bytes(y));
            continue;
        }
        p.wgrad = conv_resolve_wgrad(op.geom, p.st);
        p.wg_bytes = act_bytes(x) + grad_bytes(y) + wbytes;
        p.colsum = !op.bias_by_bn;
        if (!op.need_dx) continue;
        p.dgrad = conv_resolve_dgrad(op.geom, op.dgeom, p.st, op.wino_ud != nullptr);
        p.dg_bytes = grad_bytes(y) + grad_bytes(x) + wbytes;
        Op* bn = training && op.dy_to_bn >= 0 && e->stat_max > 0 ? &tw.ops[op.dy_to_bn] : nullptr;
        if (bn != nullptr && bn->fuse_pool >= 0 && (bn->xwin == nullptr || x.batch_stride != (int64_t)x.H * x.W * x.C)) bn = nullptr;
        if (bn == nullptr) continue;
        const bool bx = tw.t[bn->in].d_bf16;
        int blocks = -1;
        if (p.dgrad.path == DG_BF16_STORED && x.g_bf16 && bx && conv_bf16_halo_ok(op.dgeom)) blocks = conv_bf16_stat_blocks(op.dgeom);
        if (p.dgrad.path == DG_WINO && !x.g_bf16 && !bx && conv_wino_ok(op.dgeom)) blocks = conv_wino_stat_blocks(op.dgeom);
        if (blocks < 0) continue;
        if (!fits(op, blocks, op.dgeom.Cout)) return L3_ESTATE;
        p.bwd_bn = op.dy_to_bn;
        bn->bp.bwd_blocks = blocks;
    }
    for (auto& op : tw.ops) {
        if (op.kind != OP_BN) continue;
        const Tensor &x = tw.t[op.in], &y = tw.t[op.out];
        const Tensor& out = op.fuse_pool >= 0 ? tw.t[tw.ops[op.fuse_pool].out] : y;
        BnPlan& p = op.bp;
        p.stats = !training ? BS_MOVING : p.stat_blocks > 0 ? BS_PARTIALS : op.prerelu || x.d_bf16 ? BS_FAST : BS_PLAIN;
        p.bwd = training && op.fused_first ? BB_BY_FIRST_CONV : !bn_fast_ok(x.C) ? BB_PLAIN : op.fuse_pool >= 0 ? BB_FAST_POOLED
                : defers(op) ? BB_FAST_DEFERRED : BB_FAST;
        p.fwd_bytes = (!training ? 0.0 : p.stat_blocks > 0 ? (double)p.stat_blocks * 2 * x.C * 4 : act_bytes(x)) + act_bytes(x) + act_bytes(out);
        if (p.bwd == BB_BY_FIRST_CONV) p.fwd_bytes += act_bytes(x) + (double)x.rows() * (&op + 1)->ageom.Cin * 4.0;
        if (op.fuse_pool >= 0 && training && op.xwin != nullptr) p.fwd_bytes += (double)out.numel() * (x.d_bf16 ? 2.0 : 4.0);
        p.bwd_bytes = p.bwd == BB_PLAIN ? 2.0 * (act_bytes(x) + grad_bytes(y)) + grad_bytes(x)
                                        : (p.bwd_blocks > 0 ? (double)p.bwd_blocks * 2 * x.C * 4 : act_bytes(x) + grad_bytes(out)) +
                                              (p.bwd == BB_FAST_DEFERRED ? 0.0 : act_bytes(x) + grad_bytes(out) + grad_bytes(x));
    }
    return L3_OK;
}

void tower_forward(l3_engine* e, Tower& tw) {
    const bool training = tw.training;
    for (auto& op : tw.ops) {
        Tensor& x = tw.t[op.in];
        Tensor& y = tw.t[op.out];
        switch (op.kind) {
            case OP_CONV: {
                const ConvPlan& p = op.cp;
                ConvBufs b;
                b.x = x.d, b.w = e->params[op.p_kernel].d, b.bias = e->params[op.p_bias].d, b.y = y.d;
                b.wprep = op.wflip, b.wino_u = op.wino_uf;
                b.stat_part = p.stat_mode ? e->stat_scratch : nullptr, b.stat_mode = p.stat_mode;
                ProfScope ps(e, F_CONV_FWD, conv_flops(op.geom), op.name.c_str(), p.fwd.executed);
                ps.bytes(p.fwd_bytes);
                conv_run_fwd(p.fwd, op.geom, p.st, b, e->stream);
                break;
            }
            case OP_BN: {
                const BnPlan& p = op.bp;
                ProfScope ps(e, F_ELEMWISE, 0.0);
                ps.bytes(p.fwd_bytes);
                const float* gamma = e->params[op.p_gamma].d;
                const float* beta = e->params[op.p_beta].d;
                switch (p.stats) {
                    case BS_PARTIALS:
                        bn_stats_from_partials(e->stat_scratch, p.stat_blocks, e->params[op.bias_param].d, gamma, beta, op.mean, op.var,
                                               op.scale, op.shift, x.rows(), x.C, BN_EPS, op.prerelu ? 1 : 0, e->stream);
                        break;
                    case BS_FAST:
                        bn_stats_fast(x.d, gamma, beta, op.mean, op.var, op.scale, op.shift, e->red_scratch, x.rows(), x.C, BN_EPS,
                                      op.prerelu ? 1 : 0, e->stream, x.d_bf16 ? 1 : 0);
                        break;
                    case BS_PLAIN:
                        bn_stats(x.d, gamma, beta, op.mean, op.var, op.scale, op.shift, e->red_scratch, x.rows(), x.C, BN_EPS, e->stream);
                        break;
                    case BS_MOVING:
                        bn_scale_shift(gamma, beta, e->params[op.p_mmean].d, e->params[op.p_mvar].d, op.scale, op.shift, x.C, BN_EPS,
                                       e->stream);
                        break;
                }
                if (p.bwd == BB_BY_FIRST_CONV) bn_xhat_ones(x.d, op.mean, op.var, BN_EPS, (&op + 1)->xaug, x.rows(), x.C, e->stream);
                if (op.fuse_pool >= 0) {
                    Tensor& pl = tw.t[tw.ops[op.fuse_pool].out];
                    bn_relu_pool2_fwd(x.d, op.scale, op.shift, pl.d, x.N, x.H, x.W, x.C, pl.H, pl.W, pl.batch_stride,
                                      op.prerelu ? 2 : (op.fused_relu ? 1 : 0), e->stream, pl.d_bf16 ? 1 : 0, x.d_bf16 ? 1 : 0,
                                      training ? (void*)op.xwin : nullptr);
                } else if (y.d_bf16 || x.d_bf16) {
                    bn_apply_fast(x.d, op.scale, op.shift, y.d, x.rows(), x.C, op.fused_relu ? 1 : 0, e->stream, y.d_bf16 ? 1 : 0,
                                  x.d_bf16 ? 1 : 0);
                } else {
                    bn_apply(x.d, op.scale, op.shift, y.d, x.rows(), x.C, op.fused_relu ? 1 : 0, e->stream);
                }
                break;
            }
            case OP_RELU: {
                if (op.fused_into_bn) break;
                ProfScope ps(e, F_ELEMWISE, 0.0);
                ps.bytes(act_bytes(x) + act_bytes(y));
                relu_fwd(x.d, y.d, x.numel(), e->stream);
                break;
            }
            case OP_POOL: {
                if (op.fused_into_bn) break;
                ProfScope ps(e, F_ELEMWISE, 0.0);
                ps.bytes(act_bytes(x) + act_bytes(y));
                maxpool_fwd(x.d, y.d, op.pg, e->stream);
                break;
            }
            default: break;
        }
    }
}

BnBwdFuse bn_bwd_fuse(const Tower& tw, const Op& bn) {
    return BnBwdFuse{bn.fuse_pool >= 0 ? bn.xwin : tw.t[bn.in].d, bn.scale, bn.shift, bn.mean, bn.var, BN_EPS, bn.fused_relu ? 1 : 0};
}

void tower_backward_block(l3_engine* e, Tower& tw, int block) {
    const bool training = tw.training;
    for (int oi = (int)tw.ops.size() - 1; oi >= 0; --oi) {
        Op& op = tw.ops[oi];
        if (op.block != block) continue;
        Tensor& x = tw.t[op.in];
        Tensor& y = tw.t[op.out];
        switch (op.kind) {
            case OP_POOL: {
                if (op.fused_into_bn) break;
                ProfScope ps(e, F_ELEMWISE, 0.0);
                ps.bytes(act_bytes(x) + grad_bytes(y) + grad_bytes(x));
                maxpool_bwd(x.d, y.g, x.g, op.pg, e->stream);
                break;
            }
            case OP_RELU: {
                if (op.fused_into_bn) break;
                ProfScope ps(e, F_ELEMWISE, 0.0);
                ps.bytes(act_bytes(y) + grad_bytes(y) + grad_bytes(x));
                relu_bwd(y.d, y.g, x.g, x.numel(), e->stream);
                break;
            }
            case OP_BN: {
                const BnPlan& p = op.bp;
                if (p.bwd == BB_BY_FIRST_CONV) break;
                ProfScope ps(e, F_ELEMWISE, 0.0);
                ps.bytes(p.bwd_bytes);
                const float* mean = training ? op.mean : e->params[op.p_mmean].d;
                const float* var = training ? op.var : e->params[op.p_mvar].d;
                const float* gamma = e->params[op.p_gamma].d;
                float *dgamma = e->params[op.p_gamma].g, *dbeta = e->params[op.p_beta].g;
                if (p.bwd == BB_PLAIN) {
                    bn_bwd(x.d, y.d, y.g, gamma, mean, var, x.g, dgamma, dbeta, e->red_scratch, x.rows(), x.C, BN_EPS, op.fused_relu ? 1 : 0,
                           training ? 1 : 0, e->stream);
                    break;
                }
                const bool pooled = p.bwd == BB_FAST_POOLED, defer = p.bwd == BB_FAST_DEFERRED;
                const Tensor& dy = pooled ? tw.t[tw.ops[op.fuse_pool].out] : y;
                bn_bwd_fast(x.d, op.scale, op.shift, mean, var, gamma, dy.g, pooled ? 1 : 0, x.N, x.H, x.W, x.C, dy.H, dy.W,
                            pooled ? dy.batch_stride : (int64_t)x.H * x.W * x.C, defer ? nullptr : x.g, dgamma, dbeta,
                            defer ? nullptr : op.bias_param >= 0 ? e->params[op.bias_param].g : nullptr, e->red_scratch, BN_EPS,
                            pooled ? (op.prerelu ? 2 : 1) : (op.fused_relu ? 1 : 0), training ? 1 : 0, e->stream, x.g_bf16 ? 1 : 0,
                            x.d_bf16 ? 1 : 0, dy.g_bf16 ? 1 : 0, p.bwd_blocks > 0 ? e->stat_scratch : nullptr, p.bwd_blocks);
                break;
            }
            case OP_CONV: {
                const ConvPlan& p = op.cp;
                const float* w = e->params[op.p_kernel].d;
                if (p.aug != FW_NONE) {
                    ProfScope ps(e, F_CONV_WGRAD, conv_flops(op.geom), op.name.c_str());
                    ps.bytes(p.wg_bytes);
                    const Op& bn = tw.ops[op.in_bn];
                    if (p.aug == FW_AUG_DEFERRED) {
                        const Op& fb = tw.ops[op.bn_defer];
                        const Tensor &bi = tw.t[fb.in], &bo = tw.t[fb.out];
                        const float* co = bn_bwd_fast_coeffs(e->red_scratch, op.cout);
                        const FirstWgFuse f{bi.d, bo.g, fb.scale, fb.shift, co, co + op.cout, co + 2 * op.cout, fb.fused_relu ? 1 : 0,
                                            bi.d_bf16 ? 1 : 0};
                        conv_wgrad(op.xaug, nullptr, op.gaug, e->wg_scratch, op.ageom, e->stream, false, false, &f);
                    } else {
                        conv_wgrad(op.xaug, y.g, op.gaug, e->wg_scratch, op.ageom, e->stream);
                    }
                    first_conv_grads(op.gaug, w, e->params[bn.p_gamma].d, e->params[bn.p_beta].d, e->params[op.p_kernel].g,
                                     e->params[bn.p_gamma].g, e->params[bn.p_beta].g,
                                     op.bias_by_bn && p.aug == FW_AUG ? nullptr : e->params[op.p_bias].g, op.kh * op.kw, x.C, op.cout,
                                     e->stream);
                    break;
                }
                ConvBufs b;
                b.x = x.d, b.w = w, b.y = y.g, b.dx = x.g, b.dw = e->params[op.p_kernel].g;
                b.wprep = op.wflip, b.wino_u = op.wino_ud, b.wg_part = e->wg_scratch;
                {
                    ProfScope ps(e, F_CONV_WGRAD, conv_flops(op.geom), op.name.c_str(), p.wgrad.executed);
                    ps.bytes(p.wg_bytes);
                    conv_run_wgrad(p.wgrad, op.geom, b, e->stream);
                }
                if (p.colsum) {
                    ProfScope ps(e, F_ELEMWISE, 0.0);
                    ps.bytes(grad_bytes(y));
                    colsum(y.g, e->params[op.p_bias].g, e->red_scratch, y.rows(), y.C, e->stream);
                }
                if (p.dgrad.path == DG_NONE) break;
                ProfScope ps(e, F_CONV_DGRAD, conv_flops(op.geom), op.name.c_str(), p.dgrad.executed);
                ps.bytes(p.dg_bytes);
                BnBwdFuse bb{};
                if (p.bwd_bn >= 0) {
                    bb = bn_bwd_fuse(tw, tw.ops[p.bwd_bn]);
                    b.bn_bwd = &bb, b.stat_part = e->stat_scratch;
                }
                conv_run_dgrad(p.dgrad, op.geom, op.dgeom, p.st, b, e->stream);
                break;
            }
            default: break;
        }
    }
}

void l2_sums(l3_engine* e) {
    SumsqSegs segs{};
    int nl2 = 0;
    for (auto& s : e->segments) nl2 += s.l2 ? 1 : 0;
    if (nl2 <= SUMSQ_MAX_SEGS) {
        for (auto& s : e->segments)
            if (s.l2) {
                segs.off[segs.count] = s.off;
                segs.n[segs.count++] = s.n;
            }
        sumsq_multi(e->arena_p, segs, e->l2part, e->sq_scratch, e->stream);
        return;
    }
    int si = 0;
    for (auto& s : e->segments)
        if (s.l2) sumsq(e->arena_p + s.off, s.n, e->l2part + si++, e->sq_scratch, e->stream);
}

int forward_all(l3_engine* e, bool training) {
    int rc;
    e->fwd_done = false;
    if ((rc = plan_tower(e, e->vis, training, 0)) || (rc = plan_tower(e, e->aud, training, 0))) return rc;
    if (e->side && e->overlap) {
        HIPCHK(e, hipEventRecord(e->ev_fork, e->stream));
        HIPCHK(e, hipStreamWaitEvent(e->side, e->ev_fork, 0));
        l2_sums(e);
        {
            SideScope sd(e);
            if ((rc = run_frontend(e))) return rc;
            tower_forward(e, e->aud);
            HIPCHK(e, hipEventRecord(e->ev_join, e->stream));
        }
        tower_forward(e, e->vis);
        HIPCHK(e, hipStreamWaitEvent(e->stream, e->ev_join, 0));
    } else {
        l2_sums(e);
        if ((rc = run_frontend(e))) return rc;
        tower_forward(e, e->vis);
        tower_forward(e, e->aud);
    }
    ProfScope ps(e, F_HEAD, 0.0);
    const int D = e->nv + e->na;
    dense_fwd(e->h0, e->params[e->p_w1].d, e->params[e->p_b1].d, e->h1, e->B, D, e->head, 1, e->stream);
    dense_fwd(e->h1, e->params[e->p_w2].d, e->params[e->p_b2].d, e->logits, e->B, e->head, 2, 0, e->stream);
    e->last_training = training;
    return L3_OK;
}

void loss_and_head_backward(l3_engine* e, bool backward) {
    ProfScope ps(e, F_HEAD, 0.0);
    const int gb = e->cfg.global_batch > 0 ? e->cfg.global_batch : e->B;
    softmax_ce(e->logits, e->labels, e->probs, e->dlogits, e->stats, e->B, 1.0f / (float)gb, e->stream);
    if (!backward) return;
    const int D = e->nv + e->na;
    dense_bwd_w(e->h1, e->dlogits, e->params[e->p_w2].g, e->params[e->p_b2].g, e->B, e->head, 2, e->stream);
    dense_bwd_x(e->dlogits, e->params[e->p_w2].d, e->dh1, e->B, e->head, 2, e->stream);
    relu_bwd(e->h1, e->dh1, e->dh1, (int64_t)e->B * e->head, e->stream);
// ... 1314 lines not shown
```

l3embedding_amd/csrc/kernels.h:

```cpp
#pragma once
#include <hip/hip_runtime.h>
#include <stdint.h>

#include <string>
#include <vector>

#include "host_common.h"

namespace l3 {

struct ConvGeom {
    int N, H, W, Cin;
    int Ho, Wo, Cout;
    int KH, KW, padT, padL;
    int f2x2 = 0;
    int solo = 0;
    int dynamic = 0;
    float* tail_scratch = nullptr;
    size_t tail_scratch_bytes = 0;
};
size_t conv_wino4_tail_scratch_bytes();

struct BnBwdFuse {
    const float* x;
    const float *scale, *shift;
    const float *mean, *var;
    float eps;
    int relu;
};
void conv_fwd(const float* x, const float* w, const float* bias, float* y, const ConvGeom& g,
              hipStream_t s, const float* wino_u = nullptr, float* bn_part = nullptr, int bn_mode = 0,
              const BnBwdFuse* bn_bwd = nullptr);
bool conv_wino_ok(const ConvGeom& g);
size_t conv_wino_floats(const ConvGeom& g);
double conv_wino_executed_flops(const ConvGeom& g);
void conv_wino_transform_weights(const float* w, float* u, const ConvGeom& g, bool from_fwd_for_dgrad, hipStream_t s);
void conv_wino_fwd(const float* x, const float* u, const float* bias, float* y, const ConvGeom& g, hipStream_t s,
                   float* stat_part = nullptr, int stat_mode = 0, const BnBwdFuse* bn_bwd = nullptr);
int conv_wino_stat_blocks(const ConvGeom& g);
int conv_wino_stat_blocks_max(const ConvGeom& g);
bool conv_dgrad_small_ok(const ConvGeom& g);
bool conv_dgrad_small(const float* dy, const float* w, float* dx, const ConvGeom& g, hipStream_t s);
void conv_flip_weights(const float* w, float* wt, int KH, int KW, int Cin, int Cout, hipStream_t s);
size_t conv_wgrad_scratch_floats(const ConvGeom& g);
bool conv_wgrad_bf16_ok(const ConvGeom& g);
struct FirstWgFuse;
void conv_wgrad(const float* x, const float* dy, float* dw, float* part, const ConvGeom& g,
                hipStream_t s, bool bf16 = false, bool in_bf16 = false, const FirstWgFuse* first_fuse = nullptr);

bool conv_first_ok(const ConvGeom& g);
bool conv_first_wgrad_ok(const ConvGeom& g);
size_t conv_first_wgrad_scratch_floats(const ConvGeom& g);
struct FirstWgFuse {
    const void *bnx, *dA;
    const float *scale, *shift;
    const float *cA, *cB, *cC;
    int relu;
    int bf16;
};
int conv_first_wgrad(const float* x, const float* dy, float* part, const ConvGeom& g, hipStream_t s, const FirstWgFuse* fuse = nullptr);
int conv_first_stat_blocks(const ConvGeom& g);
void conv_first_fwd(const float* x, const float* w, const float* bias, void* y, const ConvGeom& g, hipStream_t s,
                    float* stat_part = nullptr, int stat_mode = 0, bool out_bf16 = false);

bool conv_wgrad_wino_ok(const ConvGeom& g);
int conv_wgrad_wino_splits(const ConvGeom& g, int n);
int conv_wgrad_wino_max_splits(const ConvGeom& g, int n);
double conv_wgrad_wino_executed_flops(const ConvGeom& g);
void conv_wgrad_wino_launch(const float* x, const float* dy, float* part, const ConvGeom& g, int n, hipStream_t s);
void conv_wgrad_wino_finish(const float* part, float* dw, const ConvGeom& g, int splits, hipStream_t s);
double conv_wgrad_executed_flops(const ConvGeom& g, bool bf16);
bool conv_wgrad_bf16_tr_enabled();
void conv_wgrad_bf16_tr_launch(const void* x, const void* dy, float* part, const ConvGeom& g, int n, int splits, hipStream_t s);

bool conv_bf16_ok(const ConvGeom& g);
void conv_bf16_fwd(const float* x, const float* wn, const float* bias, float* y, const ConvGeom& g, hipStream_t s,
                   bool operands_bf16 = false, float* stat_part = nullptr, int stat_mode = 0, bool out_bf16 = false,
                   const BnBwdFuse* bn_bwd = nullptr);
int conv_bf16_stat_blocks(const ConvGeom& g);
bool conv_bf16_halo_ok(const ConvGeom& g);
int conv_bf16_halo_patches(const ConvGeom& g, int n);
void conv_bf16_halo_launch(const void* x, const void* wn, const float* bias, void* y, const ConvGeom& g, int n,
                           hipStream_t s, float* stat_part, int stat_mode, bool out_bf16, const BnBwdFuse* bn_bwd = nullptr);
void conv_weights_bf16(const float* w, void* out, int KH, int KW, int Cin, int Cout, bool flip, hipStream_t s);

void bn_xhat_ones(const float* x, const float* mean, const float* var, float eps, float* xa, int64_t rows, int C,
                  hipStream_t s);
void first_conv_grads(const float* gaug, const float* w, const float* gamma, const float* beta, float* dw, float* dgamma,
                      float* dbeta, float* dbias, int taps, int C, int Co, hipStream_t s);

size_t colreduce_scratch_floats(int64_t rows, int C);
void colsum(const float* x, float* out, float* scratch, int64_t rows, int C, hipStream_t s);
void bn_stats(const float* x, const float* gamma, const float* beta, float* mean, float* var,
              float* scale, float* shift, float* scratch, int64_t rows, int C, float eps,
              hipStream_t s);
void bn_scale_shift(const float* gamma, const float* beta, const float* mean, const float* var,
                    float* scale, float* shift, int C, float eps, hipStream_t s);
void bn_apply(const float* x, const float* scale, const float* shift, float* y, int64_t rows, int C,
              int relu, hipStream_t s);
void bn_bwd(const float* x, const float* y, const float* dy, const float* gamma, const float* mean,
            const float* var, float* dx, float* dgamma, float* dbeta, float* scratch, int64_t rows,
            int C, float eps, int relu, int training, hipStream_t s);
void bn_moving_update(float* moving, float* biased, const float* batch, int C, float momentum,
                      int zero_debias, int step, hipStream_t s);
int* persistent_work_counters(hipStream_t s);

struct BnMovingEntry {
    float* moving;
    float* biased;
    const float* batch;
    int C;
    int off;
};
void bn_moving_update_all(const BnMovingEntry* tab_dev, int entries, int max_c, float momentum, int zero_debias, int64_t step,
                          hipStream_t s, const float* gathered = nullptr, int replicas = 1, int64_t stride = 0);
void bn_moving_pack(const BnMovingEntry* tab_dev, int entries, int max_c, float* packed, hipStream_t s);

bool bn_fast_ok(int C);
size_t bn_fast_scratch_floats(int C);
void bn_stats_fast(const float* x, const float* gamma, const float* beta, float* mean, float* var, float* scale,
                   float* shift, float* scratch, int64_t rows, int C, float eps, int prerelu, hipStream_t s, int x_bf16 = 0);
void bn_stats_from_partials(const float* part, int nblk, const float* pivot, const float* gamma, const float* beta,
                            float* mean, float* var, float* scale, float* shift, int64_t rows, int C, float eps,
                            int prerelu, hipStream_t s);
void bn_apply_fast(const float* x, const float* scale, const float* shift, float* y, int64_t rows, int C, int relu,
                   hipStream_t s, int out_bf16 = 0, int x_bf16 = 0);
void bn_relu_pool2_fwd(const float* x, const float* scale, const float* shift, float* p, int N, int H, int W, int C,
                       int Ho, int Wo, int64_t out_batch_stride, int mode, hipStream_t s, int out_bf16 = 0, int x_bf16 = 0,
                       void* xwin = nullptr);
void bn_bwd_fast(const float* x, const float* scale, const float* shift, const float* mean, const float* var,
                 const float* gamma, const float* dy, int pooled, int N, int H, int W, int C, int Ho, int Wo,
                 int64_t dy_batch_stride, float* dx, float* dgamma, float* dbeta, float* dbias, float* scratch,
                 float eps, int relu, int training, hipStream_t s, int dx_bf16 = 0, int x_bf16 = 0, int dy_bf16 = 0,
                 const float* ready_part = nullptr, int ready_blocks = 0);
const float* bn_bwd_fast_coeffs(const float* scratch, int C);

void relu_fwd(const float* x, float* y, int64_t n, hipStream_t s);
void relu_bwd(const float* y, const float* dy, float* dx, int64_t n, hipStream_t s);

struct PoolGeom {
    int N, H, W, C, Ho, Wo, ph, pw, sh, sw, padT, padL;
    int64_t out_batch_stride;
};
void maxpool_fwd(const float* x, float* y, const PoolGeom& g, hipStream_t s);
void maxpool_bwd(const float* x, const float* dy, float* dx, const PoolGeom& g, hipStream_t s);

void preprocess_video(const uint8_t* u8, float* out, int64_t n, hipStream_t s);
void preprocess_audio(const int16_t* pcm, float* out, int64_t n, hipStream_t s);
void labels_onehot(const int32_t* lab, float* out, int64_t n, hipStream_t s);

struct AugmentParams {
    int32_t start_x, start_y, flip, sat_first;
    float saturation, brightness;
};
constexpr int AUG_CROP = 224;
void augment_video(const uint8_t* u8, int N, int H, int W, const AugmentParams* params, uint8_t* out_u8, float* out_f32,
                   hipStream_t s);
void augment_audio(const int16_t* pcm, int N, int T, const double* u, int16_t* out_i16, float* out_f32, double* gains,
                   hipStream_t s);

struct FrontendCfg {
    int n_dft, n_hop, pad_left, n_frames, n_freq, n_mels;
    int sqrt_out;
    int db;
    int loglambda;
    int ncols_pad;
    int folded, ke, ko, nc;
    int factored, N1, N2;
};
void dft_pack_frames(const float* audio, const float* win, float* a1, int B, int T, const FrontendCfg& c, hipStream_t s);
void dft_twiddle(const float* y, const float* tw, float* a2, float* nyq, int frames, const FrontendCfg& c, hipStream_t s);
void frame_audio_folded(const float* audio, float* fe, float* fo, int B, int T, const FrontendCfg& c, hipStream_t s);
void frame_audio(const float* audio, float* frames, int B, int T, const FrontendCfg& c, hipStream_t s);
void dft_fused(const float* audio, const float* win, const float* b1, const float* b2, const float* tw, const float* melw,
               const int* mel_start, const int* mel_len, const int* mel_off, float* out, int B, int T, const FrontendCfg& c,
               hipStream_t s);
void spec_to_features(const float* spec, const float* melw, const int* mel_start, const int* mel_len,
                      const int* mel_off, float* out, int B, const FrontendCfg& c, hipStream_t s, const float* nyq = nullptr);
void db_normalize(float* x, float* smax, int B, int64_t per_sample, int batch_scope, hipStream_t s);

void gather_frames(const float* samples, const int64_t* table, float* out, int rows, int n_real, int T, hipStream_t s);
inline const char* frame_table_error(const int64_t* table, int64_t n_frames, int64_t n_samples, int64_t* bad_row) {
    const int64_t lim = (int64_t)1 << 62;
    for (int64_t r = 0; r < n_frames; ++r) {
        const int64_t start = table[3 * r], lo = table[3 * r + 1], hi = table[3 * r + 2];
        *bad_row = r;
        if (lo < 0) return "lo < 0";
        if (lo > hi) return "lo > hi";
        if (hi > n_samples) return "hi > n_samples";
        if (start < -lim || start > lim) return "start out of range";
    }
    return nullptr;
}

constexpr int RESAMPLE_ROW = 6;
struct ResampleClip {
    int64_t x_off, L, sr_o, sr_n, t0, n_out, y_off;
    int64_t table;
};
struct ResamplePlan {
    std::vector<ResampleClip> clips;
    std::vector<int64_t> blocks;
};
struct ResampleTables {
    std::vector<double> window;
    std::vector<double> keys;
    std::vector<double> tables;
    uint64_t generation = 0;
};
int64_t resample_out_len(int64_t L, int64_t sr_o, int64_t sr_n);
const char* resample_clips_error(const int64_t* clips, int64_t n_clips, int64_t n_native, int64_t sr_new, int64_t n_window,
                                 int num_table, int64_t n_samples, bool copy_equal, int64_t* bad);
struct ResampleStage {
    int run(const float* native, int64_t n_native, const int64_t* clips, int64_t n_clips, int64_t sr_new,
            const double* half_window, int64_t n_window, int num_table, bool copy_equal, float* d_out, int64_t n_samples,
            hipStream_t s, std::string* err);

// ... 30 lines not shown
```

l3embedding_amd/csrc/ops.hip:

```cpp
#include <hip/hip_runtime.h>

#include <cstring>
#include <string>
#include <vector>

#include "../../include/l3hip.h"
#include "conv_path.h"
#include "kernels.h"
#include "knobs.h"
#include "mlp.h"
#include "vggish.h"

namespace {
using namespace l3;

struct Scope {
    DeviceBufs bufs;
    hipStream_t s = nullptr;
    bool ok = true;
    explicit Scope(int device) : ok(device_ok(device)) {}
    ~Scope() { (void)hipDeviceSynchronize(); }
    template <class T>
    T* alloc(size_t count) {
        T* p = bufs.alloc<T>(count);
// ... 49 lines not shown

extern "C" {

int l3_op_conv2d_fwd_dt(int device, int dtype, const float* x, const float* w, const float* b, float* y, int n, int h,
                        int wd, int cin, int cout, int kh, int kw, int same) {
    Scope sc(device);
    if (!sc.ok) return L3_EHIP;
    const ConvGeom g = make_geom(n, h, wd, cin, cout, kh, kw, same);
    const size_t nx = (size_t)n * h * wd * cin, nw = (size_t)kh * kw * cin * cout, ny = (size_t)n * g.Ho * g.Wo * cout;
    const bool stored = dtype == L3_OP_BF16_STORED || dtype == L3_OP_BF16_STORED_OUT;
    ConvStorage st;
    st.mixed = dtype != L3_DTYPE_F32;
    st.x_bf16 = stored && conv_bf16_ok(g);
    const ConvFwdPath p = conv_resolve_fwd(g, st, conv_wino_floats(g) != 0);
    st.y_bf16 = dtype == L3_OP_BF16_STORED_OUT && (p.path == CF_BF16_STORED || p.path == CF_FIRST);
    ConvBufs cb;
    float* d_x = sc.put(x, nx);
    cb.x = d_x;
    cb.w = sc.put(w, nw);
    cb.bias = b ? sc.put(b, (size_t)cout) : nullptr;
    cb.y = sc.alloc<float>(ny);
    cb.wprep = sc.alloc<float>(nw);
    cb.wino_u = p.wino_filter ? sc.alloc<float>(conv_wino_floats(g)) : nullptr;
    uint16_t* xb = st.x_bf16 ? sc.alloc<uint16_t>(nx) : nullptr;
    if (!sc.ok) return L3_ENOMEM;
    if (st.x_bf16) {
        cast_bf16(d_x, xb, (int64_t)nx, sc.s);
        cb.x = reinterpret_cast<const float*>(xb);
    }
    conv_run_fwd(p, g, st, cb, sc.s);
    sc.get_stored(y, cb.y, ny, st.y_bf16);
    return sc.status();
}

int l3_op_conv2d_fwd(int device, const float* x, const float* w, const float* b, float* y, int n, int h, int wd,
                     int cin, int cout, int kh, int kw, int same) {
    return l3_op_conv2d_fwd_dt(device, L3_DTYPE_F32, x, w, b, y, n, h, wd, cin, cout, kh, kw, same);
}

int l3_op_conv2d_bwd_dt(int device, int dtype, const float* x, const float* w, const float* dy, float* dx, float* dw,
                        float* db, int n, int h, int wd, int cin, int cout, int kh, int kw, int same) {
    Scope sc(device);
    if (!sc.ok) return L3_EHIP;
    const ConvGeom g = make_geom(n, h, wd, cin, cout, kh, kw, same), dg = conv_dgrad_geom(g);
    const size_t nx = (size_t)n * h * wd * cin, ny = (size_t)n * g.Ho * g.Wo * cout, nw = (size_t)kh * kw * cin * cout;
    const bool stored = (dtype == L3_OP_BF16_STORED || dtype == L3_OP_BF16_STORED_OUT) && conv_wgrad_bf16_ok(g) && conv_bf16_ok(dg);
    ConvStorage st;
    st.mixed = dtype != L3_DTYPE_F32;
    st.x_bf16 = st.dy_bf16 = stored;
    st.dx_bf16 = stored && dtype == L3_OP_BF16_STORED_OUT;
    const ConvWgradPath pw = conv_resolve_wgrad(g, st);
    const ConvDgradPath pd = conv_resolve_dgrad(g, dg, st, conv_wino_floats(dg) != 0);
    ConvBufs cb;
    float* d_x = sc.put(x, nx);
    float* d_dy = sc.put(dy, ny);
    cb.x = d_x;
    cb.y = d_dy;
    cb.w = sc.put(w, nw);
    cb.dx = sc.alloc<float>(nx);
    cb.dw = sc.alloc<float>(nw);
    cb.wprep = sc.alloc<float>(nw);
    cb.wino_u = pd.path == DG_WINO ? sc.alloc<float>(conv_wino_floats(dg)) : nullptr;
    cb.wg_part = sc.alloc<float>(conv_wgrad_scratch_floats(g));
    float* d_db = sc.alloc<float>((size_t)cout);
    float* d_red = sc.alloc<float>(colreduce_scratch_floats((int64_t)n * g.Ho * g.Wo, cout));
    uint16_t* xb = stored ? sc.alloc<uint16_t>(nx) : nullptr;
    uint16_t* gb = stored ? sc.alloc<uint16_t>(ny) : nullptr;
    if (!sc.ok) return L3_ENOMEM;
    if (stored) {
        cast_bf16(d_x, xb, (int64_t)nx, sc.s);
        cast_bf16(d_dy, gb, (int64_t)ny, sc.s);
        cb.x = reinterpret_cast<const float*>(xb);
        cb.y = reinterpret_cast<float*>(gb);
    }
    conv_run_wgrad(pw, g, cb, sc.s);
    colsum(d_dy, d_db, d_red, (int64_t)n * g.Ho * g.Wo, cout, sc.s);
    conv_run_dgrad(pd, g, dg, st, cb, sc.s);
    sc.get_stored(dx, cb.dx, nx, st.dx_bf16);
    sc.get(dw, cb.dw, nw);
    sc.get(db, d_db, (size_t)cout);
    return sc.status();
}

int l3_op_conv2d_bwd(int device, const float* x, const float* w, const float* dy, float* dx, float* dw, float* db,
                     int n, int h, int wd, int cin, int cout, int kh, int kw, int same) {
    return l3_op_conv2d_bwd_dt(device, L3_DTYPE_F32, x, w, dy, dx, dw, db, n, h, wd, cin, cout, kh, kw, same);
}

int l3_op_bn_relu_fwd(int device, const float* x, const float* gamma, const float* beta, float* y, float* mean,
                      float* var, int64_t rows, int c, int relu, int x_bf16) {
    Scope sc(device);
    if (!sc.ok) return L3_EHIP;
    if ((x_bf16 & 1) && !bn_fast_ok(c)) return L3_EINVAL;
    const size_t n = (size_t)rows * c, cp = (size_t)(c + 3) / 4 * 4;
    float* d_x = sc.put(x, n);
    float* d_g = sc.alloc<float>(cp);
    float* d_b = sc.alloc<float>(cp);
    float *d_m = sc.alloc<float>(cp), *d_v = sc.alloc<float>(cp), *d_sc = sc.alloc<float>(cp), *d_sh = sc.alloc<float>(cp);
    float* d_y = sc.alloc<float>(n);
    float* d_red = sc.alloc<float>(colreduce_scratch_floats(rows, c));
    if (!sc.ok) return L3_ENOMEM;
    (void)hipMemcpy(d_g, gamma, c * 4, hipMemcpyHostToDevice);
    (void)hipMemcpy(d_b, beta, c * 4, hipMemcpyHostToDevice);
    if (x_bf16 & 1) {
        uint16_t* xb = sc.alloc<uint16_t>(n);
        if (!sc.ok) return L3_ENOMEM;
        cast_bf16(d_x, xb, (int64_t)n, sc.s);
        bn_stats_fast(reinterpret_cast<const float*>(xb), d_g, d_b, d_m, d_v, d_sc, d_sh, d_red, rows, c, 1e-3f, 0, sc.s, 1);
        bn_apply_fast(reinterpret_cast<const float*>(xb), d_sc, d_sh, d_y, rows, c, relu, sc.s, 0, 1);
    } else {
        bn_stats(d_x, d_g, d_b, d_m, d_v, d_sc, d_sh, d_red, rows, c, 1e-3f, sc.s);
        bn_apply(d_x, d_sc, d_sh, d_y, rows, c, relu, sc.s);
    }
    sc.get(y, d_y, n);
    sc.get(mean, d_m, (size_t)c);
    sc.get(var, d_v, (size_t)c);
    return sc.status();
}

int l3_op_bn_relu_bwd(int device, const float* x, const float* y, const float* dy, const float* gamma,
                      const float* beta, const float* mean, const float* var, float* dx, float* dgamma, float* dbeta,
                      int64_t rows, int c, int relu, int x_bf16) {
    Scope sc(device);
    if (!sc.ok) return L3_EHIP;
    const size_t n = (size_t)rows * c, cp = (size_t)(c + 3) / 4 * 4;
    float* d_x = sc.put(x, n);
    float* d_y = sc.put(y, n);
    float* d_dy = sc.put(dy, n);
    float *d_g = sc.alloc<float>(cp), *d_m = sc.alloc<float>(cp), *d_v = sc.alloc<float>(cp);
    float *d_dg = sc.alloc<float>(cp), *d_db = sc.alloc<float>(cp);
    float* d_dx = sc.alloc<float>(n);
    const bool fast = beta != nullptr && bn_fast_ok(c) && rows < (int64_t)1 << 30;
    if (x_bf16 && !fast) return L3_EINVAL;
    size_t red = colreduce_scratch_floats(rows, c);
    if (fast && bn_fast_scratch_floats(c) > red) red = bn_fast_scratch_floats(c);
    float* d_red = sc.alloc<float>(red);
    if (!sc.ok) return L3_ENOMEM;
    (void)hipMemcpy(d_g, gamma, c * 4, hipMemcpyHostToDevice);
    (void)hipMemcpy(d_m, mean, c * 4, hipMemcpyHostToDevice);
    (void)hipMemcpy(d_v, var, c * 4, hipMemcpyHostToDevice);
    if (fast) {
        float *d_b = sc.put(beta, (size_t)c), *d_sc = sc.alloc<float>(cp), *d_sh = sc.alloc<float>(cp);
        if (!sc.ok) return L3_ENOMEM;
        bn_scale_shift(d_g, d_b, d_m, d_v, d_sc, d_sh, c, 1e-3f, sc.s);
        const float* xin = d_x;
        const float* dyin = d_dy;
        if (x_bf16 & 1) {
            uint16_t* xb = sc.alloc<uint16_t>(n);
            if (!sc.ok) return L3_ENOMEM;
            cast_bf16(d_x, xb, (int64_t)n, sc.s);
            xin = reinterpret_cast<const float*>(xb);
        }
        if (x_bf16 & 2) {
            uint16_t* gb = sc.alloc<uint16_t>(n);
            if (!sc.ok) return L3_ENOMEM;
            cast_bf16(d_dy, gb, (int64_t)n, sc.s);
            dyin = reinterpret_cast<const float*>(gb);
        }
        bn_bwd_fast(xin, d_sc, d_sh, d_m, d_v, d_g, dyin, 0, 1, 1, (int)rows, c, 1, (int)rows, (int64_t)rows * c, d_dx, d_dg,
                    d_db, nullptr, d_red, 1e-3f, relu, 1, sc.s, 0, (x_bf16 & 1) ? 1 : 0, (x_bf16 & 2) ? 1 : 0);
    } else {
        bn_bwd(d_x, d_y, d_dy, d_g, d_m, d_v, d_dx, d_dg, d_db, d_red, rows, c, 1e-3f, relu, 1, sc.s);
    }
    sc.get(dx, d_dx, n);
    sc.get(dgamma, d_dg, (size_t)c);
    sc.get(dbeta, d_db, (size_t)c);
// ... 746 lines not shown
```

Baseline: 2006 pairs/s.

## Fuse Winograd wgrad split-reduce with finish and carry deferred BN bias sum

On the Winograd fp32 weight-gradient path, the split reduction and the G^T·G finish transform now run in a single kernel instead of a reduce kernel followed by a finish kernel. When the following BN backward produces the conv bias gradient and nothing runs between them, that final bias column-sum is deferred and computed by extra blocks inside the same fused launch. The aim is fewer kernel launches and no round trip of the summed 16-slice buffer through HBM. The cost is a more complex engine planning step and a fixed 1024-thread block shape for the reduction.

```diff
diff --git a/include/l3hip.h b/include/l3hip.h
--- a/include/l3hip.h
+++ b/include/l3hip.h
@@ -143,6 +143,7 @@
 int l3_op_conv2d_bwd(int device, const float *x, const float *w, const float *dy,
                      float *dx, float *dw, float *db,
                      int n, int h, int wd, int cin, int cout, int kh, int kw, int same);
+int l3_op_conv_wgrad_slices(int n, int h, int wd, int cin, int cout, int kh, int kw, int same, int *slices, int *groups);
 int l3_op_bn_relu_fwd(int device, const float *x, const float *gamma, const float *beta,
                       float *y, float *mean, float *var, int64_t rows, int c, int relu, int x_bf16);
 int l3_op_bn_relu_bwd(int device, const float *x, const float *y, const float *dy,
diff --git a/l3embedding_amd/_lib.py b/l3embedding_amd/_lib.py
--- a/l3embedding_amd/_lib.py
+++ b/l3embedding_amd/_lib.py
@@ -116,6 +116,7 @@
     'l3_op_conv2d_fwd_dt': (C.c_int, [C.c_int, C.c_int, C.c_void_p, C.c_void_p, C.c_void_p, C.c_void_p] + [C.c_int] * 8),
     'l3_op_conv2d_bwd_dt': (C.c_int, [C.c_int, C.c_int] + [C.c_void_p] * 6 + [C.c_int] * 8),
     'l3_op_conv2d_bwd': (C.c_int, [C.c_int] + [C.c_void_p] * 6 + [C.c_int] * 8),
+    'l3_op_conv_wgrad_slices': (C.c_int, [C.c_int] * 8 + [C.POINTER(C.c_int)] * 2),
     'l3_op_bn_relu_fwd': (C.c_int, [C.c_int] + [C.c_void_p] * 6 + [C.c_int64, C.c_int, C.c_int, C.c_int]),
     'l3_op_bn_relu_bwd': (C.c_int, [C.c_int] + [C.c_void_p] * 10 + [C.c_int64, C.c_int, C.c_int, C.c_int]),
     'l3_op_bn_relu_pool2_fwd': (C.c_int, [C.c_int] + [C.c_void_p] * 6 + [C.c_int] * 7),
@@ -634,6 +635,12 @@
     return dx, dw, db
 
 
+def op_conv_wgrad_slices(n, h, wd, cin, cout, kh=3, kw=3, same=True):
+    slices, groups = C.c_int(0), C.c_int(0)
+    check(load().l3_op_conv_wgrad_slices(n, h, wd, cin, cout, kh, kw, int(same), C.byref(slices), C.byref(groups)))
+    return slices.value, groups.value
+
+
 def op_bn_relu_fwd(x, gamma, beta, relu, device=0, x_bf16=False):
     lib = load()
     x = _f32(x)
diff --git a/l3embedding_amd/csrc/bn_fused.hip b/l3embedding_amd/csrc/bn_fused.hip
--- a/l3embedding_amd/csrc/bn_fused.hip
+++ b/l3embedding_amd/csrc/bn_fused.hip
@@ -1,5 +1,6 @@
 #include "kernels.h"
 #include "device_common.h"
+#include "fast_final.h"
 
 namespace l3 {
 
@@ -92,23 +93,7 @@
     const int lane = threadIdx.x & 63, wave = threadIdx.x >> 6;
     const int c = blockIdx.x * 4 + wave;
     if (c >= C) return;
-    double s0 = 0.0, s1 = 0.0;
-    for (int b = lane; b < nblk; b += 64) {
-        if constexpr (PRE) {
-            const double* row = reinterpret_cast<const double*>(part + (size_t)b * rpb * 2 * C);
-            s0 += row[c];
-            s1 += row[C + c];
-        } else {
-            s0 += (double)part[((size_t)b * 2 + 0) * C + c];
-            s1 += (double)part[((size_t)b * 2 + 1) * C + c];
-        }
-    }
-#pragma unroll
-    for (int off = 32; off > 0; off >>= 1) {
-        s0 += __shfl_xor(s0, off, 64);
-        s1 += __shfl_xor(s1, off, 64);
-    }
-    if (lane == 0) g(c, s0, s1);
+    fast_final_channel<G, PRE>(g, part, nblk, C, rpb, c, lane);
 }
 
 constexpr int PRE_BLOCKS = 256;
@@ -544,16 +529,13 @@
     if (part != nullptr) block_write_partials(a0, a0, part, g.C4);
 }
 
-struct SumFinal {
-    float* out;
-    __device__ void operator()(int c, double s0, double) const { out[c] = (float)s0; }
-};
+void bn_sum_final(const DeferredSum& d, hipStream_t s) { launch_fast_final(SumFinal{d.out}, d.part, d.nblk, d.C, s); }
 
 void bn_bwd_fast(const float* x, const float* scale, const float* shift, const float* mean, const float* var,
                  const float* gamma, const float* dy, int pooled, int N, int H, int W, int C, int Ho, int Wo,
                  int64_t dy_batch_stride, float* dx, float* dgamma, float* dbeta, float* dbias, float* scratch,
                  float eps, int relu, int training, hipStream_t s, int dx_bf16, int x_bf16, int dy_bf16,
-                 const float* ready_part, int ready_blocks) {
+                 const float* ready_part, int ready_blocks, DeferredSum* defer_dbias) {
     const int64_t rows = (int64_t)N * H * W;
     const int64_t n4 = rows * (C / 4);
     Pool2Geom g = make_pool2(N, H, W, C, pooled ? Ho : H, pooled ? Wo : W, pooled ? dy_batch_stride : (int64_t)H * W * C);
@@ -598,7 +580,12 @@
     hipLaunchKernelGGL(apply_fns[variant], dim3(nb_a), dim3(FB), 0, s, xv, dyv, sc4, sh4, reinterpret_cast<const f32x4*>(cA),
                        reinterpret_cast<const f32x4*>(cB), reinterpret_cast<const f32x4*>(cC), (void*)dx, part2, n4, g, relu,
                        dx_bf16);
-    if (dbias) launch_fast_final(SumFinal{dbias}, part, nb_a, C, s);
-}
-
-}
+    if (!dbias) return;
+    const DeferredSum sum{part, nb_a, C, dbias};
+    if (defer_dbias != nullptr)
+        *defer_dbias = sum;
+    else
+        bn_sum_final(sum, s);
+}
+
+}
diff --git a/l3embedding_amd/csrc/conv.hip b/l3embedding_amd/csrc/conv.hip
--- a/l3embedding_amd/csrc/conv.hip
+++ b/l3embedding_amd/csrc/conv.hip
@@ -766,13 +766,19 @@
     }
 }
 
+int wgrad_reduce_groups(int64_t n4, int splits) {
+    if (n4 < 1024 && splits >= 256) return 64;
+    return n4 / 64 >= 1024 || splits < 16 ? 4 : 16;
+}
+
 static void wgrad_reduce(const float* part, float* dw, int64_t n, int splits, hipStream_t s) {
     if (n % 4 == 0 && splits > 1) {
         const int64_t n4 = n / 4;
-        if (n4 < 1024 && splits >= 256)
+        const int sg = wgrad_reduce_groups(n4, splits);
+        if (sg == 64)
             hipLaunchKernelGGL(wgrad_reduce4_kernel<64>, dim3((unsigned)((n4 + 3) / 4)), dim3(256), 0, s,
                                reinterpret_cast<const f32x4*>(part), reinterpret_cast<f32x4*>(dw), n4, splits);
-        else if (n4 / 64 >= 1024 || splits < 16)
+        else if (sg == 4)
             hipLaunchKernelGGL(wgrad_reduce4_kernel<4>, dim3((unsigned)((n4 + 63) / 64)), dim3(256), 0, s,
                                reinterpret_cast<const f32x4*>(part), reinterpret_cast<f32x4*>(dw), n4, splits);
         else
@@ -1168,6 +1174,13 @@
     return total;
 }
 
+int conv_wgrad_wino_total_splits(const ConvGeom& g) {
+    const int nc = wgrad9_chunk_samples(g);
+    int total = 0;
+    for (int n0 = 0; n0 < g.N; n0 += nc) total += conv_wgrad_wino_splits(g, g.N - n0 < nc ? g.N - n0 : nc);
+    return total;
+}
+
 size_t conv_wgrad_scratch_floats(const ConvGeom& g) {
     if (wgrad9_ok(g)) {
         const size_t direct = (size_t)wgrad9_total_splits(g) * 9 * g.Cin * g.Cout;
@@ -1183,17 +1196,20 @@
     return wgrad9_ok(g) && (size_t)g.H * g.W * (g.Cin > g.Cout ? g.Cin : g.Cout) * 4 + (size_t)(g.W + 1) * g.Cin * 4 < (1ull << 31);
 }
 
+bool conv_wgrad_wino_path(const ConvGeom& g) { return wgrad9_ok(g) && conv_wgrad_bf16_ok(g) && conv_wgrad_wino_ok(g); }
+
 double conv_wgrad_executed_flops(const ConvGeom& g, bool bf16) {
-    if (!bf16 && wgrad9_ok(g) && conv_wgrad_bf16_ok(g) && conv_wgrad_wino_ok(g)) return conv_wgrad_wino_executed_flops(g);
+    if (!bf16 && conv_wgrad_wino_path(g)) return conv_wgrad_wino_executed_flops(g);
     return -1.0;
 }
 
 void conv_wgrad(const float* x, const float* dy, float* dw, float* part, const ConvGeom& g,
-                hipStream_t s, bool bf16, bool in_bf16, const FirstWgFuse* first_fuse) {
+                hipStream_t s, bool bf16, bool in_bf16, const FirstWgFuse* first_fuse, bool fused_finish,
+                const DeferredSum* carry) {
     if (wgrad9_ok(g)) {
         static const int use_t = l3_knob("L3_WG9T") ? atoi(l3_knob("L3_WG9T")) : 1;
         const bool fits = conv_wgrad_bf16_ok(g);
-        if (!bf16 && fits && conv_wgrad_wino_ok(g)) {
+        if (!bf16 && conv_wgrad_wino_path(g)) {
             const int nc = wgrad9_chunk_samples(g);
             const size_t slice = (size_t)16 * g.Cin * g.Cout;
             int total = 0;
@@ -1202,6 +1218,10 @@
                 conv_wgrad_wino_launch(x + (size_t)n0 * g.H * g.W * g.Cin, dy + (size_t)n0 * g.H * g.W * g.Cout,
                                        part + (size_t)total * slice, g, n, s);
                 total += conv_wgrad_wino_splits(g, n);
+            }
+            if (fused_finish) {
+                conv_wgrad_wino_reduce_finish(part, dw, g, total, carry, s);
+                return;
             }
             float* sum = part + (size_t)total * slice;
             if (total > 1) wgrad_reduce(part, sum, (int64_t)slice, total, s);
diff --git a/l3embedding_amd/csrc/conv_path.h b/l3embedding_amd/csrc/conv_path.h
--- a/l3embedding_amd/csrc/conv_path.h
+++ b/l3embedding_amd/csrc/conv_path.h
@@ -21,6 +21,7 @@
 };
 struct ConvWgradPath {
     ConvWgrad path = WG_FP32;
+    bool fused_finish = false;
     double executed = -1.0;
 };
 struct ConvDgradPath {
@@ -45,6 +46,7 @@
     float* stat_part = nullptr;
     int stat_mode = 0;
     const BnBwdFuse* bn_bwd = nullptr;
+    const DeferredSum* bias_sum = nullptr;
 };
 void conv_run_fwd(const ConvFwdPath& p, const ConvGeom& g, const ConvStorage& st, const ConvBufs& b, hipStream_t s);
 void conv_run_wgrad(const ConvWgradPath& p, const ConvGeom& g, const ConvBufs& b, hipStream_t s);
diff --git a/l3embedding_amd/csrc/conv_path.hip b/l3embedding_amd/csrc/conv_path.hip
--- a/l3embedding_amd/csrc/conv_path.hip
+++ b/l3embedding_amd/csrc/conv_path.hip
@@ -1,4 +1,5 @@
 #include "conv_path.h"
+#include "knobs.h"
 
 namespace l3 {
 
@@ -36,6 +37,7 @@
     const bool wbf = st.mixed && conv_wgrad_bf16_ok(g);
     p.path = !wbf ? WG_FP32 : st.x_bf16 && st.dy_bf16 ? WG_BF16_STORED : WG_BF16_CAST;
     p.executed = conv_wgrad_executed_flops(g, wbf);
+    p.fused_finish = !wbf && conv_wgrad_wino_path(g) && knob_int("L3_WGW_FUSED_FINISH", 1) != 0;
     return p;
 }
 
@@ -68,7 +70,9 @@
 }
 
 void conv_run_wgrad(const ConvWgradPath& p, const ConvGeom& g, const ConvBufs& b, hipStream_t s) {
-    conv_wgrad(b.x, b.y, b.dw, b.wg_part, g, s, p.path != WG_FP32, p.path == WG_BF16_STORED);
+    conv_wgrad(b.x, b.y, b.dw, b.wg_part, g, s, p.path != WG_FP32, p.path == WG_BF16_STORED, nullptr, p.fused_finish,
+               p.fused_finish ? b.bias_sum : nullptr);
+    if (b.bias_sum != nullptr && !p.fused_finish) bn_sum_final(*b.bias_sum, s);
 }
 
 void conv_run_dgrad(const ConvDgradPath& p, const ConvGeom& g, const ConvGeom& dg, const ConvStorage& st, const ConvBufs& b, hipStream_t s) {
diff --git a/l3embedding_amd/csrc/conv_wgrad_wino.hip b/l3embedding_amd/csrc/conv_wgrad_wino.hip
--- a/l3embedding_amd/csrc/conv_wgrad_wino.hip
+++ b/l3embedding_amd/csrc/conv_wgrad_wino.hip
@@ -1,6 +1,7 @@
 #include "kernels.h"
 #include "device_common.h"
 #include "wgw_common.h"
+#include "fast_final.h"
 
 #include <stdlib.h>
 
@@ -235,6 +236,24 @@
         }
 }
 
+__device__ __forceinline__ void wgw_gtg_store(const float (&u)[16], float* __restrict__ dw, int cc, int idx) {
+    float rrow[3][4];
+#pragma unroll
+    for (int nu = 0; nu < 4; ++nu) {
+        const float h1 = 0.5f * u[4 + nu], h2 = 0.5f * u[8 + nu];
+        rrow[0][nu] = u[nu] + (h1 + h2);
+        rrow[1][nu] = h1 - h2;
+        rrow[2][nu] = (h1 + h2) + u[12 + nu];
+    }
+#pragma unroll
+    for (int kh = 0; kh < 3; ++kh) {
+        const float h1 = 0.5f * rrow[kh][1], h2 = 0.5f * rrow[kh][2];
+        dw[(size_t)(kh * 3 + 0) * cc + idx] = rrow[kh][0] + (h1 + h2);
+        dw[(size_t)(kh * 3 + 1) * cc + idx] = h1 - h2;
+        dw[(size_t)(kh * 3 + 2) * cc + idx] = (h1 + h2) + rrow[kh][3];
+    }
+}
+
 __global__ __launch_bounds__(256) void wgw_finish_kernel(const float* __restrict__ part, float* __restrict__ dw, int cc,
                                                          int splits) {
     const int idx = blockIdx.x * 256 + threadIdx.x;
@@ -245,20 +264,41 @@
     for (int s = 0; s < splits; ++s)
 #pragma unroll
         for (int p = 0; p < 16; ++p) u[p] += __builtin_nontemporal_load(part + ((size_t)s * 16 + p) * cc + idx);
-    float rrow[3][4];
-#pragma unroll
-    for (int nu = 0; nu < 4; ++nu) {
-        const float h1 = 0.5f * u[4 + nu], h2 = 0.5f * u[8 + nu];
-        rrow[0][nu] = u[nu] + (h1 + h2);
-        rrow[1][nu] = h1 - h2;
-        rrow[2][nu] = (h1 + h2) + u[12 + nu];
-    }
-#pragma unroll
-    for (int kh = 0; kh < 3; ++kh) {
-        const float h1 = 0.5f * rrow[kh][1], h2 = 0.5f * rrow[kh][2];
-        dw[(size_t)(kh * 3 + 0) * cc + idx] = rrow[kh][0] + (h1 + h2);
-        dw[(size_t)(kh * 3 + 1) * cc + idx] = h1 - h2;
-        dw[(size_t)(kh * 3 + 2) * cc + idx] = (h1 + h2) + rrow[kh][3];
+    wgw_gtg_store(u, dw, cc, idx);
+}
+
+template <int SG>
+__global__ __launch_bounds__(1024) void wgw_reduce_finish_kernel(const f32x4* __restrict__ part, float* __restrict__ dw, int cc,
+                                                                 int total, int cblocks, DeferredSum carry) {
+    constexpr int COLS = 1024 / (16 * SG);
+    const int t = threadIdx.x;
+    if ((int)blockIdx.x < cblocks) {
+        const int c = blockIdx.x * 16 + (t >> 6);
+        if (c < carry.C) fast_final_channel<SumFinal, false>(SumFinal{carry.out}, carry.part, carry.nblk, carry.C, 1, c, t & 63);
+        return;
+    }
+    __shared__ f32x4 red[1024];
+    const int blk = blockIdx.x - cblocks;
+    const int q = t % COLS, p = (t / COLS) % 16, g = t / (COLS * 16);
+    const int cc4 = cc / 4;
+    const int64_t n4 = (int64_t)16 * cc4;
+    const f32x4* src = part + (int64_t)p * cc4 + (blk * COLS + q);
+    f32x4 s = {0.f, 0.f, 0.f, 0.f};
+    for (int sp = g; sp < total; sp += SG) s += __builtin_nontemporal_load(src + (int64_t)sp * n4);
+    red[t] = s;
+    __syncthreads();
+    if (g == 0) {
+#pragma unroll
+        for (int k = 1; k < SG; ++k) s += red[(k * 16 + p) * COLS + q];
+        red[t] = s;
+    }
+    __syncthreads();
+    if (t < 4 * COLS) {
+        const float* f = reinterpret_cast<const float*>(red);
+        float u[16];
+#pragma unroll
+        for (int pp = 0; pp < 16; ++pp) u[pp] = f[pp * 4 * COLS + t];
+        wgw_gtg_store(u, dw, cc, blk * 4 * COLS + t);
     }
 }
 
@@ -358,4 +398,17 @@
     hipLaunchKernelGGL(wgw_finish_kernel, dim3((cc + 255) / 256), dim3(256), 0, s, part, dw, cc, splits);
 }
 
-}
+void conv_wgrad_wino_reduce_finish(const float* part, float* dw, const ConvGeom& g, int total, const DeferredSum* carry,
+                                   hipStream_t s) {
+    const int cc = g.Cin * g.Cout, cc4 = cc / 4;
+    const int sg = wgrad_reduce_groups((int64_t)16 * cc4, total);
+    const DeferredSum c = carry != nullptr ? *carry : DeferredSum{};
+    const int cblocks = (c.C + 15) / 16;
+    const f32x4* p4 = reinterpret_cast<const f32x4*>(part);
+    if (sg == 16)
+        hipLaunchKernelGGL(wgw_reduce_finish_kernel<16>, dim3(cblocks + cc4 / 4), dim3(1024), 0, s, p4, dw, cc, total, cblocks, c);
+    else
+        hipLaunchKernelGGL(wgw_reduce_finish_kernel<4>, dim3(cblocks + cc4 / 16), dim3(1024), 0, s, p4, dw, cc, total, cblocks, c);
+}
+
+}
diff --git a/l3embedding_amd/csrc/engine.hip b/l3embedding_amd/csrc/engine.hip
--- a/l3embedding_amd/csrc/engine.hip
+++ b/l3embedding_amd/csrc/engine.hip
@@ -61,6 +61,7 @@
     FirstWgrad aug = FW_NONE;
     ConvWgradPath wgrad;
     bool colsum = false;
+    bool carry_bias = false;
     ConvDgradPath dgrad;
     int bwd_bn = -1;
     double fwd_bytes = 0.0, wg_bytes = 0.0, dg_bytes = 0.0;
@@ -72,6 +73,7 @@
     int stat_blocks = 0;
     BnBwd bwd = BB_PLAIN;
     int bwd_blocks = 0;
+    bool defer_bias = false;
     double fwd_bytes = 0.0, bwd_bytes = 0.0;
 };
 
@@ -106,6 +108,7 @@
     bool bias_by_bn = false;
     float *mean = nullptr, *var = nullptr, *scale = nullptr, *shift = nullptr;
     float *biased_mean = nullptr, *biased_var = nullptr;
+    DeferredSum bias_sum{};
     PoolGeom pg{};
     ConvPlan cp{};
     BnPlan bp{};
@@ -1209,6 +1212,16 @@
                                         : (p.bwd_blocks > 0 ? (double)p.bwd_blocks * 2 * x.C * 4 : act_bytes(x) + grad_bytes(out)) +
                                               (p.bwd == BB_FAST_DEFERRED ? 0.0 : act_bytes(x) + grad_bytes(out) + grad_bytes(x));
     }
+    for (size_t i = 0; i < tw.ops.size(); ++i) {
+        Op& cv = tw.ops[i];
+        if (cv.kind != OP_CONV || cv.cp.aug != FW_NONE || !cv.cp.wgrad.fused_finish || cv.bn_follow <= (int)i || !cv.bias_by_bn) continue;
+        Op& bn = tw.ops[cv.bn_follow];
+        if (bn.block != cv.block || bn.bias_param < 0 || bn.bias_param != cv.p_bias) continue;
+        if (bn.bp.bwd != BB_FAST && bn.bp.bwd != BB_FAST_POOLED) continue;
+        bool idle = true;
+        for (int k = (int)i + 1; k < cv.bn_follow; ++k) idle = idle && tw.ops[k].fused_into_bn;
+        if (idle) cv.cp.carry_bias = bn.bp.defer_bias = true;
+    }
     return L3_OK;
 }
 
@@ -1327,11 +1340,13 @@
                 }
                 const bool pooled = p.bwd == BB_FAST_POOLED, defer = p.bwd == BB_FAST_DEFERRED;
                 const Tensor& dy = pooled ? tw.t[tw.ops[op.fuse_pool].out] : y;
+                op.bias_sum = DeferredSum{};
                 bn_bwd_fast(x.d, op.scale, op.shift, mean, var, gamma, dy.g, pooled ? 1 : 0, x.N, x.H, x.W, x.C, dy.H, dy.W,
                             pooled ? dy.batch_stride : (int64_t)x.H * x.W * x.C, defer ? nullptr : x.g, dgamma, dbeta,
                             defer ? nullptr : op.bias_param >= 0 ? e->params[op.bias_param].g : nullptr, e->red_scratch, BN_EPS,
                             pooled ? (op.prerelu ? 2 : 1) : (op.fused_relu ? 1 : 0), training ? 1 : 0, e->stream, x.g_bf16 ? 1 : 0,
-                            x.d_bf16 ? 1 : 0, dy.g_bf16 ? 1 : 0, p.bwd_blocks > 0 ? e->stat_scratch : nullptr, p.bwd_blocks);
+                            x.d_bf16 ? 1 : 0, dy.g_bf16 ? 1 : 0, p.bwd_blocks > 0 ? e->stat_scratch : nullptr, p.bwd_blocks,
+                            p.defer_bias ? &op.bias_sum : nullptr);
                 break;
             }
             case OP_CONV: {
@@ -1360,6 +1375,7 @@
                 ConvBufs b;
                 b.x = x.d, b.w = w, b.y = y.g, b.dx = x.g, b.dw = e->params[op.p_kernel].g;
                 b.wprep = op.wflip, b.wino_u = op.wino_ud, b.wg_part = e->wg_scratch;
+                if (p.carry_bias) b.bias_sum = &tw.ops[op.bn_follow].bias_sum;
                 {
                     ProfScope ps(e, F_CONV_WGRAD, conv_flops(op.geom), op.name.c_str(), p.wgrad.executed);
                     ps.bytes(p.wg_bytes);
diff --git a/l3embedding_amd/csrc/fast_final.h b/l3embedding_amd/csrc/fast_final.h
--- /dev/null
+++ b/l3embedding_amd/csrc/fast_final.h
@@ -0,0 +1,32 @@
+#pragma once
+#include <hip/hip_runtime.h>
+
+namespace l3 {
+
+template <class G, bool PRE>
+__device__ __forceinline__ void fast_final_channel(const G& g, const float* part, int nblk, int C, int rpb, int c, int lane) {
+    double s0 = 0.0, s1 = 0.0;
+    for (int b = lane; b < nblk; b += 64) {
+        if constexpr (PRE) {
+            const double* row = reinterpret_cast<const double*>(part + (size_t)b * rpb * 2 * C);
+            s0 += row[c];
+            s1 += row[C + c];
+        } else {
+            s0 += (double)part[((size_t)b * 2 + 0) * C + c];
+            s1 += (double)part[((size_t)b * 2 + 1) * C + c];
+        }
+    }
+#pragma unroll
+    for (int off = 32; off > 0; off >>= 1) {
+        s0 += __shfl_xor(s0, off, 64);
+        s1 += __shfl_xor(s1, off, 64);
+    }
+    if (lane == 0) g(c, s0, s1);
+}
+
+struct SumFinal {
+    float* out;
+    __device__ void operator()(int c, double s0, double) const { out[c] = (float)s0; }
+};
+
+}
diff --git a/l3embedding_amd/csrc/kernels.h b/l3embedding_amd/csrc/kernels.h
--- a/l3embedding_amd/csrc/kernels.h
+++ b/l3embedding_amd/csrc/kernels.h
@@ -45,8 +45,17 @@
 size_t conv_wgrad_scratch_floats(const ConvGeom& g);
 bool conv_wgrad_bf16_ok(const ConvGeom& g);
 struct FirstWgFuse;
+struct DeferredSum {
+    const float* part = nullptr;
+    int nblk = 0, C = 0;
+    float* out = nullptr;
+};
 void conv_wgrad(const float* x, const float* dy, float* dw, float* part, const ConvGeom& g,
-                hipStream_t s, bool bf16 = false, bool in_bf16 = false, const FirstWgFuse* first_fuse = nullptr);
+                hipStream_t s, bool bf16 = false, bool in_bf16 = false, const FirstWgFuse* first_fuse = nullptr,
+                bool fused_finish = false, const DeferredSum* carry = nullptr);
+int wgrad_reduce_groups(int64_t n4, int splits);
+bool conv_wgrad_wino_path(const ConvGeom& g);
+int conv_wgrad_wino_total_splits(const ConvGeom& g);
 
 bool conv_first_ok(const ConvGeom& g);
 bool conv_first_wgrad_ok(const ConvGeom& g);
@@ -69,6 +78,8 @@
 double conv_wgrad_wino_executed_flops(const ConvGeom& g);
 void conv_wgrad_wino_launch(const float* x, const float* dy, float* part, const ConvGeom& g, int n, hipStream_t s);
 void conv_wgrad_wino_finish(const float* part, float* dw, const ConvGeom& g, int splits, hipStream_t s);
+void conv_wgrad_wino_reduce_finish(const float* part, float* dw, const ConvGeom& g, int total, const DeferredSum* carry,
+                                   hipStream_t s);
 double conv_wgrad_executed_flops(const ConvGeom& g, bool bf16);
 bool conv_wgrad_bf16_tr_enabled();
 void conv_wgrad_bf16_tr_launch(const void* x, const void* dy, float* part, const ConvGeom& g, int n, int splits, hipStream_t s);
@@ -132,7 +143,9 @@
                  const float* gamma, const float* dy, int pooled, int N, int H, int W, int C, int Ho, int Wo,
                  int64_t dy_batch_stride, float* dx, float* dgamma, float* dbeta, float* dbias, float* scratch,
                  float eps, int relu, int training, hipStream_t s, int dx_bf16 = 0, int x_bf16 = 0, int dy_bf16 = 0,
-                 const float* ready_part = nullptr, int ready_blocks = 0);
+                 const float* ready_part = nullptr, int ready_blocks = 0,
+                 DeferredSum* defer_dbias = nullptr);
+void bn_sum_final(const DeferredSum& d, hipStream_t s);
 const float* bn_bwd_fast_coeffs(const float* scratch, int C);
 
 void relu_fwd(const float* x, float* y, int64_t n, hipStream_t s);
diff --git a/l3embedding_amd/csrc/ops.hip b/l3embedding_amd/csrc/ops.hip
--- a/l3embedding_amd/csrc/ops.hip
+++ b/l3embedding_amd/csrc/ops.hip
@@ -155,6 +155,14 @@
     return sc.status();
 }
 
+int l3_op_conv_wgrad_slices(int n, int h, int wd, int cin, int cout, int kh, int kw, int same, int* slices, int* groups) {
+    const ConvGeom g = make_geom(n, h, wd, cin, cout, kh, kw, same);
+    const bool wino = conv_wgrad_wino_path(g);
+    *slices = wino ? conv_wgrad_wino_total_splits(g) : 0;
+    *groups = wino ? wgrad_reduce_groups((int64_t)4 * cin * cout, *slices) : 0;
+    return L3_OK;
+}
+
 int l3_op_conv2d_bwd(int device, const float* x, const float* w, const float* dy, float* dx, float* dw, float* db,
                      int n, int h, int wd, int cin, int cout, int kh, int kw, int same) {
     return l3_op_conv2d_bwd_dt(device, L3_DTYPE_F32, x, w, dy, dx, dw, db, n, h, wd, cin, cout, kh, kw, same);
```

Result: no change. 2002 pairs/s (median of 2 runs) (-0.2%).
